# victorvg17/Towards-Interpretable-Reinforcement-Learning-Using-Attention-Augmented-Agents-Replication

Hardware: AMD Instinct MI355X
Metric: learner frames/sec (fwd+bwd, T=20 unroll) at 1/2/4/8 MI355X + % roofline (higher is better)
Workload: dtype fp32; 1 GPU; C2 (BASELINE.json configs[1]): B=32 per GPU x T=20 unroll, 84x84, 4 heads, fp32; global_batch=32, seq_len=20, frame=84x84, heads=4, parallelism=dp1

## Files before the change

### include/aaa.h

```cpp
#ifndef AAA_H
#define AAA_H

#include <stddef.h>
#include <hip/hip_runtime_api.h>

#ifdef __cplusplus
extern "C" {
#endif

#define AAA_ABI_VERSION 11

enum aaa_status {
  AAA_OK = 0,
  AAA_E_ARG = -1,
  AAA_E_ALIGN = -2,
  AAA_E_LAUNCH = -3,
  AAA_E_DEVICE = -4,
  AAA_E_STRANDED = -5
};

enum aaa_dtype {
  AAA_F32 = 0,
  AAA_BF16 = 1
};
// ... 171 lines not shown
  const void* packed;
  const float* basis;
  const void* frames;
  const float* prev_reward;
  const float* prev_action;
  float* h;
  float* c;
  float* logits;
  float* values;
  float* attn;
  void* workspace;
  unsigned long long seed;
  unsigned long long* counter;
  int* actions;
  float* logp;
  float* dlogp_dlogits;
  float* gates;
  float* h_out;
  float* c_out;
} aaa_actor_io;
size_t aaa_actor_workspace_bytes(const aaa_cfg* cfg);
int aaa_actor_step(const aaa_cfg* cfg, const aaa_actor_io* io, hipStream_t stream);

typedef struct aaa_actor_core_io {
  float* core_h;
  float* core_c;
  float* core_h_out;
  float* core_c_out;
  float* query;
} aaa_actor_core_io;
size_t aaa_actor_core_workspace_bytes(const aaa_cfg* cfg);
int aaa_actor_step_core(const aaa_cfg* cfg, const aaa_actor_io* io, const aaa_actor_core_io* core,
                        hipStream_t stream);


typedef struct aaa_conv_desc {
  int N, Hin, Win, Cin, Hout, Wout, Cout, KH, KW, stride, pad, dtype;
} aaa_conv_desc;

int aaa_conv2d_nhwc(const aaa_conv_desc* d, const float* x, const float* w, const float* bias,
                    float* y, hipStream_t stream);
int aaa_conv2d_nhwc_dgrad(const aaa_conv_desc* d, const float* dy, const float* w, float* dx,
                          hipStream_t stream);
int aaa_conv2d_nhwc_wgrad(const aaa_conv_desc* d, const float* x, const float* dy, float* dw,
                          hipStream_t stream);

int aaa_linear(int M, int N, int K, const float* x, const float* w, const float* bias, float* y,
               hipStream_t stream);


typedef struct aaa_cell_desc {
  int B, h, w, dtype;
} aaa_cell_desc;
size_t aaa_convlstm_packed_bytes(const aaa_cell_desc* d);
size_t aaa_convlstm_workspace_bytes(const aaa_cell_desc* d);
int aaa_convlstm_pack(const aaa_cell_desc* d, const float* cell_params, void* packed, hipStream_t stream);
int aaa_convlstm_cell_fwd(const aaa_cell_desc* d, const void* packed, const float* x, const float* h0,
                          const float* c0, float* h1, float* c1, void* workspace, hipStream_t stream);
int aaa_convlstm_cell_bwd(const aaa_cell_desc* d, const void* packed, const float* dh1, const float* dc1, float* dx,
                          float* dh0, float* dc0, float* cell_grads, void* workspace, hipStream_t stream);

typedef struct aaa_cnn_desc {
  int N, H, W, dtype;
} aaa_cnn_desc;
size_t aaa_vision_cnn_packed_bytes(const aaa_cnn_desc* d);
size_t aaa_vision_cnn_workspace_bytes(const aaa_cnn_desc* d);
int aaa_vision_cnn_pack(const aaa_cnn_desc* d, const float* cnn_params, void* packed, hipStream_t stream);
int aaa_vision_cnn_fwd(const aaa_cnn_desc* d, const float* cnn_params, const void* packed, const float* frames,
                       float* y1, float* y2, void* workspace, hipStream_t stream);
int aaa_vision_cnn_bwd(const aaa_cnn_desc* d, const void* packed, const float* dy2, float* dy1, float* cnn_grads,
                       void* workspace, hipStream_t stream);

typedef struct aaa_enc_desc {
  int N, H, W, dtype, flags, out_ld;
} aaa_enc_desc;
size_t aaa_vision_enc_workspace_bytes(const aaa_enc_desc* d);
int aaa_vision_enc_fwd(const aaa_enc_desc* d, const float* cnn_params, const void* packed, const void* frames,
                       void* xp, void* y1, void* out, hipStream_t stream);
int aaa_vision_enc_bwd(const aaa_enc_desc* d, const void* packed, const void* frames, const void* dy2,
                       const void* y1, void* xp, void* dy1, float* cnn_grads, int* fused, void* workspace,
                       hipStream_t stream);
int aaa_vision_enc_f32_fwd(const aaa_enc_desc* d, const float* cnn_params, const void* packed, const void* frames,
                           float* xp, float* y1, float* out, hipStream_t stream);

int aaa_attn_fwd(int F, int h, int w, int nq, const float* O, const float* S, const float* Q, int q_stride,
                 const float* prev_reward, const float* prev_action, float* attn, float* answer, hipStream_t stream);
int aaa_attn_bwd(int F, int h, int w, int nq, const float* O, const float* S, const float* Q, int q_stride,
                 const float* attn, const float* danswer, float* dO, float* dQ, hipStream_t stream);
int aaa_attn_fwd_bf16(int F, int h, int w, int nq, const void* O, int o_ld, const float* S, const float* Q,
                      int q_stride, float* sq_scratch, const float* prev_reward, const float* prev_action,
                      float* attn, float* answer, hipStream_t stream);
int aaa_attn_bwd_bf16(int F, int h, int w, int nq, const void* O, int o_ld, const float* S, const float* Q,
                      int q_stride, const float* attn, const float* danswer, int da_ld, int add_q,
                      int dO_quad_major, float* dO, float* dQ, hipStream_t stream);

int aaa_fastdiv_check(unsigned d, unsigned lo, unsigned hi, unsigned long long* mismatches);
int aaa_divisor_log(int enable, unsigned* out, int cap);

#ifdef __cplusplus
}
#endif
#endif
```

### towards-interpretable-reinforcement-learning-using-attention-augmented-agents-replication_amd/_native.py

```python
from __future__ import annotations

import ctypes
import os
import threading

_HERE = os.path.dirname(os.path.abspath(__file__))
LIB_PATH = os.environ.get("AAA_LIB") or os.path.join(_HERE, "libaaa.so")

F32, BF16 = 0, 1
ABI_VERSION = 11
E_STRANDED = -5
BWD_HEAD, BWD_CORE, BWD_VISION, BWD_ALL = 1, 2, 4, 7
FWD_VISION, FWD_CORE, FWD_TAIL, FWD_ALL = 1, 2, 4, 7

EXPORTS = (
    "aaa_abi_version", "aaa_last_error", "aaa_grid", "aaa_param_layout", "aaa_packed_bytes",
    "aaa_workspace_bytes", "aaa_pack_weights", "aaa_forward", "aaa_backward", "aaa_conv2d_nhwc",
    "aaa_conv2d_nhwc_dgrad", "aaa_conv2d_nhwc_wgrad", "aaa_linear", "aaa_timing_enable", "aaa_timing_read", "aaa_timing_stats",
    "aaa_adam_step", "aaa_reinforce", "aaa_sample_actions", "aaa_fastdiv_check", "aaa_divisor_log",
    "aaa_convlstm_packed_bytes", "aaa_convlstm_workspace_bytes", "aaa_convlstm_pack", "aaa_convlstm_cell_fwd",
    "aaa_convlstm_cell_bwd", "aaa_vision_cnn_packed_bytes", "aaa_vision_cnn_workspace_bytes", "aaa_vision_cnn_pack",
    "aaa_vision_cnn_fwd", "aaa_vision_cnn_bwd", "aaa_attn_fwd", "aaa_attn_bwd", "aaa_attn_fwd_bf16", "aaa_attn_bwd_bf16",
    "aaa_actor_workspace_bytes", "aaa_actor_step", "aaa_pair_status", "aaa_pair_flag", "aaa_pair_flag_at",
    "aaa_adam_step_guarded", "aaa_adam_step_counted", "aaa_workspace_region",
    "aaa_core_elem_bytes", "aaa_forward_phases", "aaa_core_export", "aaa_core_import",
    "aaa_actor_core_workspace_bytes", "aaa_actor_step_core",
    "aaa_vision_enc_workspace_bytes", "aaa_vision_enc_fwd", "aaa_vision_enc_bwd",
    "aaa_vtrace",
    "aaa_forward_resets", "aaa_backward_resets",
    "aaa_vision_enc_f32_fwd",
    "aaa_grad_norm_scratch_bytes", "aaa_grad_norm", "aaa_grad_scale", "aaa_adam_step_clipped",
)
TIMER_FWD_STEP, TIMER_BPTT_STEP, TIMER_CORE_WGRAD, TIMER_ATTN_FWD, TIMER_ATTN_BWD = 0, 1, 2, 3, 4
TIMER_PACK, TIMER_VISION_FWD, TIMER_TAIL_FWD, TIMER_TAIL_BWD, TIMER_CORE_DX, TIMER_VISION_BWD, TIMER_MISC = range(5, 12)
TIMER_N = 12


class Cfg(ctypes.Structure):
    _fields_ = [("B", ctypes.c_int), ("T", ctypes.c_int), ("H", ctypes.c_int), ("W", ctypes.c_int),
                ("nq", ctypes.c_int), ("A", ctypes.c_int), ("dtype", ctypes.c_int), ("flags", ctypes.c_int)]


IO_FIELDS = ("params", "packed", "basis", "frames", "prev_reward", "prev_action", "h0", "c0",
             "logits", "values", "attn", "hT", "cT", "dlogits", "dvalues", "dhT", "dcT",
             "grads", "dh0", "dc0", "workspace",
             "core_h0", "core_c0", "core_hT", "core_cT", "dcore_hT", "dcore_cT", "dcore_h0", "dcore_c0")
FLAG_STATEFUL_CORE = 1
FLAG_FRAMES_U8 = 2
FLAG_DEFER_STRANDED = 4
WS_ANSWER_HIDDEN, WS_QUERY_HIDDEN0, WS_QUERY_HIDDEN1 = 0, 1, 2
WS_CORE_XH, WS_CORE_DO, WS_CORE_DX = 3, 4, 5


class TimerStats(ctypes.Structure):
    _fields_ = [("total_ms", ctypes.c_double), ("launches", ctypes.c_long), ("work", ctypes.c_double),
                ("variant", ctypes.c_char * 192)]


class IO(ctypes.Structure):
    _fields_ = [(n, ctypes.c_void_p) for n in IO_FIELDS]


ACTOR_IO_FIELDS = ("params", "packed", "basis", "frames", "prev_reward", "prev_action", "h", "c",
                   "logits", "values", "attn", "workspace")


class ActorIO(ctypes.Structure):
    _fields_ = [(n, ctypes.c_void_p) for n in ACTOR_IO_FIELDS] + [
        ("seed", ctypes.c_ulonglong), ("counter", ctypes.c_void_p), ("actions", ctypes.c_void_p),
        ("logp", ctypes.c_void_p), ("dlogp_dlogits", ctypes.c_void_p), ("gates", ctypes.c_void_p),
        ("h_out", ctypes.c_void_p), ("c_out", ctypes.c_void_p)]


class ActorCoreIO(ctypes.Structure):
    _fields_ = [(n, ctypes.c_void_p) for n in ("core_h", "core_c", "core_h_out", "core_c_out", "query")]


class VtraceDesc(ctypes.Structure):
    _fields_ = [(n, ctypes.c_int) for n in ("T", "B", "A", "value_col")] + [
        (n, ctypes.c_double) for n in ("gamma", "lam", "rho_bar", "c_bar", "pg_rho_bar", "baseline_cost",
                                       "entropy_cost", "scale")]


VTRACE_IO_FIELDS = ("logits", "values", "actions", "rewards", "behaviour_logp", "done", "bootstrap",
                    "dlogits", "dvalues", "vs", "pg_adv", "loss")


class VtraceIO(ctypes.Structure):
    _fields_ = [(n, ctypes.c_void_p) for n in VTRACE_IO_FIELDS]


class AdamHP(ctypes.Structure):
    _fields_ = [("lr", ctypes.c_double), ("beta1", ctypes.c_double), ("beta2", ctypes.c_double),
                ("eps", ctypes.c_double), ("weight_decay", ctypes.c_double), ("amsgrad", ctypes.c_int),
                ("maximize", ctypes.c_int)]


class CellDesc(ctypes.Structure):
    _fields_ = [(n, ctypes.c_int) for n in ("B", "h", "w", "dtype")]


class CnnDesc(ctypes.Structure):
    _fields_ = [(n, ctypes.c_int) for n in ("N", "H", "W", "dtype")]


class EncDesc(ctypes.Structure):
    _fields_ = [(n, ctypes.c_int) for n in ("N", "H", "W", "dtype", "flags", "out_ld")]


class ConvDesc(ctypes.Structure):
    _fields_ = [(n, ctypes.c_int) for n in
                ("N", "Hin", "Win", "Cin", "Hout", "Wout", "Cout", "KH", "KW", "stride", "pad", "dtype")]


_lib = None
_lock = threading.Lock()


def ablation_build() -> bool:
    return hasattr(load(), "aaa_ablation_build")


def load(path: str = LIB_PATH):
    global _lib
    with _lock:
        if _lib is not None:
            return _lib
        if not os.path.isfile(path):
            raise RuntimeError(f"aaa: native library {path} is missing; build it with "
                               f"`make -C {os.path.join(_HERE, 'csrc')}` -- there is no CPU fallback")
        lib = ctypes.CDLL(path)
        P, I, S = ctypes.c_void_p, ctypes.c_int, ctypes.c_size_t
        CP = ctypes.POINTER(Cfg)
        sig = {
            "aaa_abi_version": (I, []),
            "aaa_last_error": (ctypes.c_char_p, []),
            "aaa_grid": (I, [I, I, ctypes.POINTER(I), ctypes.POINTER(I)]),
            "aaa_param_layout": (I, [CP, ctypes.POINTER(S), ctypes.POINTER(S), ctypes.POINTER(S)]),
            "aaa_packed_bytes": (S, [CP]),
            "aaa_workspace_bytes": (S, [CP]),
            "aaa_pack_weights": (I, [CP, P, P, P]),
            "aaa_forward": (I, [CP, ctypes.POINTER(IO), P]),
            "aaa_backward": (I, [CP, ctypes.POINTER(IO), I, P]),
            "aaa_forward_phases": (I, [CP, ctypes.POINTER(IO), I, P]),
            "aaa_forward_resets": (I, [CP, ctypes.POINTER(IO), I, P, P]),
            "aaa_backward_resets": (I, [CP, ctypes.POINTER(IO), I, P, P]),
            "aaa_core_export": (I, [CP, P, I, I, P, P, P, P]),
            "aaa_core_import": (I, [CP, P, I, I, P, P, P, P]),
            "aaa_conv2d_nhwc": (I, [ctypes.POINTER(ConvDesc), P, P, P, P, P]),
            "aaa_conv2d_nhwc_dgrad": (I, [ctypes.POINTER(ConvDesc), P, P, P, P]),
            "aaa_conv2d_nhwc_wgrad": (I, [ctypes.POINTER(ConvDesc), P, P, P, P]),
            "aaa_linear": (I, [I, I, I, P, P, P, P, P]),
            "aaa_timing_enable": (I, [I]),
            "aaa_timing_read": (I, [I, ctypes.POINTER(ctypes.c_double), ctypes.POINTER(ctypes.c_long)]),
            "aaa_timing_stats": (I, [I, ctypes.POINTER(TimerStats)]),
            "aaa_adam_step": (I, [ctypes.POINTER(AdamHP), ctypes.c_long, I, P, P, P, P, P, P, P]),
            "aaa_adam_step_guarded": (I, [ctypes.POINTER(AdamHP), ctypes.c_long, P, I, P, P, P, P, P, P, P]),
            "aaa_pair_flag": (I, [P, P]),
            "aaa_pair_flag_at": (I, [P, P, P]),
            "aaa_adam_step_counted": (I, [ctypes.POINTER(AdamHP), P, P, I, P, P, P, P, P, P, P]),
            "aaa_grad_norm_scratch_bytes": (S, [I, P]),
            "aaa_grad_norm": (I, [ctypes.c_double, I, P, P, P, P, P]),
            "aaa_grad_scale": (I, [P, I, P, P, P]),
            "aaa_adam_step_clipped": (I, [ctypes.POINTER(AdamHP), P, P, P, I, P, P, P, P, P, P, P]),
            "aaa_core_elem_bytes": (I, [ctypes.POINTER(Cfg), ctypes.POINTER(I), ctypes.POINTER(I)]),
            "aaa_workspace_region": (I, [ctypes.POINTER(Cfg), I, ctypes.POINTER(ctypes.c_size_t),
                                         ctypes.POINTER(ctypes.c_size_t)]),
            "aaa_reinforce": (I, [I, I, I, P, P, P, ctypes.c_double, P, P, P, P]),
            "aaa_vtrace": (I, [ctypes.POINTER(VtraceDesc), ctypes.POINTER(VtraceIO), P]),
            "aaa_sample_actions": (I, [I, I, P, ctypes.c_ulonglong, P, P, P, P, P]),
            "aaa_convlstm_packed_bytes": (S, [ctypes.POINTER(CellDesc)]),
            "aaa_convlstm_workspace_bytes": (S, [ctypes.POINTER(CellDesc)]),
            "aaa_convlstm_pack": (I, [ctypes.POINTER(CellDesc), P, P, P]),
            "aaa_convlstm_cell_fwd": (I, [ctypes.POINTER(CellDesc), P, P, P, P, P, P, P, P]),
            "aaa_convlstm_cell_bwd": (I, [ctypes.POINTER(CellDesc), P, P, P, P, P, P, P, P, P]),
            "aaa_vision_cnn_packed_bytes": (S, [ctypes.POINTER(CnnDesc)]),
            "aaa_vision_cnn_workspace_bytes": (S, [ctypes.POINTER(CnnDesc)]),
            "aaa_vision_cnn_pack": (I, [ctypes.POINTER(CnnDesc), P, P, P]),
            "aaa_vision_cnn_fwd": (I, [ctypes.POINTER(CnnDesc), P, P, P, P, P, P, P]),
            "aaa_vision_cnn_bwd": (I, [ctypes.POINTER(CnnDesc), P, P, P, P, P, P]),
            "aaa_vision_enc_workspace_bytes": (S, [ctypes.POINTER(EncDesc)]),
            "aaa_vision_enc_fwd": (I, [ctypes.POINTER(EncDesc), P, P, P, P, P, P, P]),
            "aaa_vision_enc_bwd": (I, [ctypes.POINTER(EncDesc), P, P, P, P, P, P, P, ctypes.POINTER(I), P, P]),
            "aaa_vision_enc_f32_fwd": (I, [ctypes.POINTER(EncDesc), P, P, P, P, P, P, P]),
            "aaa_attn_fwd": (I, [I, I, I, I, P, P, P, I, P, P, P, P, P]),
            "aaa_attn_bwd": (I, [I, I, I, I, P, P, P, I, P, P, P, P, P]),
            "aaa_attn_fwd_bf16": (I, [I, I, I, I, P, I, P, P, I, P, P, P, P, P, P]),
            "aaa_attn_bwd_bf16": (I, [I, I, I, I, P, I, P, P, I, P, P, I, I, I, P, P, P]),
            "aaa_fastdiv_check": (I, [ctypes.c_uint, ctypes.c_uint, ctypes.c_uint, ctypes.POINTER(ctypes.c_ulonglong)]),
            "aaa_divisor_log": (I, [I, ctypes.POINTER(ctypes.c_uint), I]),
            "aaa_actor_workspace_bytes": (S, [CP]),
            "aaa_actor_step": (I, [CP, ctypes.POINTER(ActorIO), P]),
            "aaa_actor_core_workspace_bytes": (S, [CP]),
            "aaa_actor_step_core": (I, [CP, ctypes.POINTER(ActorIO), ctypes.POINTER(ActorCoreIO), P]),
            "aaa_pair_status": (I, [P, I]),
        }
        ab_override = "AAA_LIB" in os.environ
        missing = [name for name in sig if not hasattr(lib, name)]
        if missing and not ab_override:
            raise RuntimeError(f"aaa: {path} does not export {missing}; it is older than these bindings -- "
                               f"rebuild it (make -C {os.path.join(_HERE, 'csrc')})")
        for name, (res, args) in sig.items():
            if name in missing:
                continue
            fn = getattr(lib, name)
            fn.restype, fn.argtypes = res, args
        abi = lib.aaa_abi_version()
        if abi != ABI_VERSION and not ab_override:
            raise RuntimeError(f"aaa: {path} has ABI version {abi}, these bindings expect {ABI_VERSION}; "
                               f"rebuild it (make -C {os.path.join(_HERE, 'csrc')})")
        _lib = lib
        return lib


def check(rc: int, what: str = "") -> None:
    if rc != 0:
        msg = load().aaa_last_error().decode(errors="replace")
        raise RuntimeError(f"aaa{(' ' + what) if what else ''}: {msg} (status {rc})")


def ptr(t) -> int | None:
    if t is None:
        return None
    return t.data_ptr()


def stream_ptr(device=None) -> int:
    import torch
    return torch.cuda.current_stream(device).cuda_stream


def grid(H: int, W: int):
    h, w = ctypes.c_int(), ctypes.c_int()
    check(load().aaa_grid(H, W, ctypes.byref(h), ctypes.byref(w)), "grid")
    return h.value, w.value


def param_layout(cfg: Cfg):
    total = ctypes.c_size_t()
    offs = (ctypes.c_size_t * 34)()
    sizes = (ctypes.c_size_t * 34)()
    check(load().aaa_param_layout(ctypes.byref(cfg), ctypes.byref(total), offs, sizes), "param_layout")
    return total.value, list(offs), list(sizes)


def fastdiv_check(d: int, lo: int = 0, hi: int = 1 << 31) -> int:
    bad = ctypes.c_ulonglong()
    check(load().aaa_fastdiv_check(d, lo, hi, ctypes.byref(bad)), "fastdiv_check")
    return bad.value


def divisor_log(enable: int = -1):
    n = load().aaa_divisor_log(-1, None, 0)
    buf = (ctypes.c_uint * max(n, 1))()
    n = load().aaa_divisor_log(enable, buf, n)
    return sorted(set(buf[:n]))


def timing_enable(on: bool = True) -> None:
    check(load().aaa_timing_enable(1 if on else 0), "timing_enable")


def timing_read(kind: int):
    ms, n = ctypes.c_double(), ctypes.c_long()
    check(load().aaa_timing_read(kind, ctypes.byref(ms), ctypes.byref(n)), "timing_read")
    return ms.value, n.value

# ... 85 lines not shown
```

### towards-interpretable-reinforcement-learning-using-attention-augmented-agents-replication_amd/csrc/misc.h

```cpp
#pragma once
#include "common.h"
#include "epilogues.h"

namespace aaa {

struct LstmPtrs {
  const float* wx[4];
  const float* bx[4];
  const float* wh[4];
};
struct LstmGrads {
  float* wx[4];
  float* bx[4];
  float* wh[4];
};
struct F32Pack {
  const float *a0w, *wih, *bih, *bhh, *pw, *vw, *pb, *vb;
  float *W1p, *Wihp, *blc, *Whd, *bhd;
  int ans_in, ans_ld, A, ldy;
  const float* whh = nullptr;
  float* Wihhp = nullptr;
};
struct F32Unpack {
  const float *gW1p, *gWihp, *gblc, *gWhd, *gbhd;
  float *a0w, *wih, *bih, *bhh, *pw, *vw, *pb, *vb;
  int ans_in, ans_ld, A;
  const float* gWihhp = nullptr;
  float* whh = nullptr;
};

template <typename T>
struct PackAll {
  const float *c1w, *c2w;
  T *Wp1, *Wp2, *WdT2;
  LstmPtrs lstm;
  T *WpX, *WpH, *WdT, *WpXH;
  float* bl;
  F32Pack f32;
  __bf16 *W1s = nullptr, *W2s = nullptr;
};
template <typename T> hipError_t pack_all(const PackAll<T>& a, hipStream_t st);
hipError_t pack_vis_split(const float* c1w, const float* c2w, __bf16* W1s, __bf16* W2s, hipStream_t st);

hipError_t query_pack(const float* b0, const float* W2, const float* b2, const float* W4, const float* b4, int nq,
                      float* q1, float* q2, float* Q, hipStream_t st);
hipError_t query_sq(const float* S, const float* Q, int P, int nq, float* SQ, hipStream_t st);
struct OSrc {
  const void* p;
  int bf16, ld;
  OSrc frame(size_t f, int P) const {
    return {(const char*)p + f * P * ld * (bf16 ? 2 : 4), bf16, ld};
  }
};
inline OSrc o_f32(const float* Hs) { return {Hs, 0, 128}; }
inline OSrc o_bf16(const __bf16* h, int ld) { return {h, 1, ld}; }
hipError_t attn_fwd(OSrc O, const float* S, const float* Q, const float* SQ, const float* pr,
                    const float* pa, int F, int P, int nq, float* Am, float* ans, int ans_ld, hipStream_t st,
                    int qs = 0);
hipError_t attn_bwd(OSrc O, const float* S, const float* Q, const float* Am, const float* dAns,
                    int da_ld, int F, int P, int nq, float* dO, float* dQp, hipStream_t st, int qs = 0,
                    int addq = 0, int cqm = 0);
hipError_t cqm_convert(const float* src, float* dst, int nf, int P, int to_cqm, hipStream_t st);
hipError_t query_bwd(const float* dQs, const float* gb1, const float* W1, int ans_in, int nq, const float* W2,
                     const float* W4, const float* q1, const float* q2, float* gW4, float* gb4, float* gW2,
                     float* gb2, float* gb0, hipStream_t st);
struct ColSumSeg {
  const float* X;
  int ld, N;
  float* out;
};
struct ColSums {
  ColSumSeg s[6];
  int n = 0;
  int cb[7];
  void add(const float* X, int ld, int N, float* out) { s[n++] = ColSumSeg{X, ld, N, out}; }
};
hipError_t colsum_multi(ColSums c, int M, hipStream_t st);
template <typename TI> hipError_t colsum(const TI* X, int ld, int M, int N, float* out, hipStream_t st);
template <typename TZ, typename GT>
hipError_t gate_bwd_last(int M, int bj, const float* dO, const float* dhT, const GT* gates, const float* cprev,
                         const float* ccur, float* dC, TZ* dz, float* part, hipStream_t st, int nsl = 1,
                         size_t sls = 0);
hipError_t concat_dy(int F, int A, int ldy, const float* dl, const float* dv, float* dY, hipStream_t st);
struct ZeroRanges {
  float* p[4];
  long n[4];
  int cnt;
  void add(float* q, long m) {
    if (q && m > 0) { p[cnt] = q; n[cnt] = m; ++cnt; }
  }
};
template <typename T>
hipError_t prologue(const ZeroRanges& z, int M, const float* h0, T* xh, int F, int A, int ldy, const float* dl,
                    const float* dv, float* dY, hipStream_t st);
template <typename T> hipError_t state_to_xh(int M, const float* h0, T* xh, hipStream_t st);
template <typename T> hipError_t xh_to_state(int M, const T* xh, float* h, hipStream_t st);
template <typename T> hipError_t cell_xh(int M, const float* x, const float* h, T* xh, hipStream_t st);
template <typename TI, typename TO> hipError_t cast(long n, const TI* src, TO* dst, hipStream_t st);
template <typename T> hipError_t pack_conv(const float* w, int Cout, int Cin, int K, T* dst, hipStream_t st);
template <typename T>
hipError_t pack_lstm_all(const LstmPtrs& L, T* WpX, T* WpH, T* WdT, float* bl, T* WpXH, hipStream_t st);
template <typename T>
hipError_t gate_fwd_zx(int M, const float* cprev, float* gates, float* cnext, float* hout, T* xhnext, hipStream_t st,
                       const float* zs = nullptr, int nsl = 0, size_t sls = 0, const float* bias = nullptr);
struct ResetZero { float* p; int ld, w, es; };
struct ResetZeros {
  ResetZero r[4];
  int n = 0;
  ResetZeros& add(float* p, int ld, int w, int es = 1) {
    if (p) r[n++] = ResetZero{p, ld, w, es};
    return *this;
  }
};
hipError_t reset_rows(const float* rs, int B, int rpb, const ResetZeros& z, const float* src, float* dst, int cw,
                      hipStream_t st);
hipError_t reset_gate_bwd(const float* rs_in, const float* rs_c, int M, int P, const float* dO, const float* gates,
                          const float* cprev, const float* ccur, float* dC, float* dz, hipStream_t st);
hipError_t pack_f32(const F32Pack& p, hipStream_t st);
hipError_t reorder_cmaj(const float* src, int rows, int Cin, int taps, int BK, float* dst, hipStream_t st);
hipError_t split_planes(const float* src, long n, __bf16* dst, hipStream_t st);
template <typename T, typename TI> hipError_t frames_rgbx(int F, int H, int W, const TI* x, T* y, hipStream_t st);
template <typename T> hipError_t pack_conv2_classes(const float* w2, T* dst, hipStream_t st);
template <typename T> hipError_t pack_conv1_rgbx(const float* w, T* dst, hipStream_t st);
hipError_t unpack_conv1_rgbx(const float* g, float* dst, hipStream_t st);
hipError_t unpack_conv(const float* g, int Cout, int Cin, int K, float* dst, hipStream_t st);
// ... 7 lines not shown
```

### towards-interpretable-reinforcement-learning-using-attention-augmented-agents-replication_amd/csrc/misc.hip

```cpp
#include <cstdlib>
#include <type_traits>

#include "misc.h"

namespace aaa {

__device__ __forceinline__ float wave_sum(float v) {
#pragma unroll
  for (int o = 32; o > 0; o >>= 1) v += __shfl_xor(v, o, 64);
  return v;
}
__device__ __forceinline__ void lds_barrier() { asm volatile("s_waitcnt lgkmcnt(0)\n\ts_barrier" ::: "memory"); }
__device__ __forceinline__ float wave_max(float v) {
#pragma unroll
  for (int o = 32; o > 0; o >>= 1) v = fmaxf(v, __shfl_xor(v, o, 64));
  return v;
}

__global__ void k_gemv_cols_atomic(const float* __restrict__ W, int ldw, const float* __restrict__ x, int N, int K,
                                   int rows_per, float* y) {
  const int o0 = blockIdx.x * rows_per, o1 = min(N, o0 + rows_per);
  for (int k = threadIdx.x; k < K; k += blockDim.x) {
    float s = 0.f;
#pragma unroll 8
// ... 793 lines not shown
        }
    } else {
      z = *reinterpret_cast<const f32x4*>(gates + (size_t)m * 512 + 4 * ch);
    }
    float gi, gf, gc, go, c, h;
    GateFwd::run(z[0], z[1], z[2], z[3], cprev[idx], gi, gf, gc, go, c, h);
    cnext[idx] = c;
    if (hout) hout[idx] = h;
    xhnext[(size_t)m * 192 + 64 + ch] = (T)h;
    *reinterpret_cast<f32x4*>(gates + (size_t)m * 512 + 4 * ch) = f32x4{gi, gf, gc, go};
  }
}

__host__ __device__ inline int pack_f32_n(const F32Pack& p) {
  return 512 * p.ans_ld + 1024 * 256 + 1024 + p.ldy * 256 + p.ldy + (p.Wihhp ? 1024 * 512 : 0);
}
__device__ __forceinline__ void pack_f32_el(int idx, const F32Pack& p) {
  const int n1 = 512 * p.ans_ld, n2 = 1024 * 256, n3 = 1024, n4 = p.ldy * 256, n5 = p.ldy;
  int i = idx;
  if (i >= n1 + n2 + n3 + n4 + n5) {
    i -= n1 + n2 + n3 + n4 + n5;
    const int row = i >> 9, k = i & 511, u = row >> 2, g = row & 3;
    p.Wihhp[i] = k < 256 ? p.wih[(size_t)(g * 256 + u) * 256 + k] : p.whh[(size_t)(g * 256 + u) * 256 + k - 256];
    return;
  }
  if (i < n1) {
    const int o = i / p.ans_ld, k = i - o * p.ans_ld;
    p.W1p[i] = k < p.ans_in ? p.a0w[(size_t)o * p.ans_in + k] : 0.f;
    return;
  }
  i -= n1;
  if (i < n2) {
    const int row = i >> 8, k = i & 255, u = row >> 2, g = row & 3;
    p.Wihp[i] = p.wih[(size_t)(g * 256 + u) * 256 + k];
    return;
  }
  i -= n2;
  if (i < n3) {
    const int u = i >> 2, g = i & 3;
    p.blc[i] = p.bih[g * 256 + u] + p.bhh[g * 256 + u];
    return;
  }
  i -= n3;
  if (i < n4) {
    const int o = i >> 8, k = i & 255;
    float v = 0.f;
    if (o < p.A) v = p.pw[o * 256 + k];
    else if (o < 2 * p.A) v = p.vw[(o - p.A) * 256 + k];
    p.Whd[i] = v;
    return;
  }
  i -= n4;
  float v = 0.f;
  if (i < p.A) v = p.pb[i];
  else if (i < 2 * p.A) v = p.vb[i - p.A];
  p.bhd[i] = v;
}
__global__ void k_pack_f32(F32Pack p) {
  const int tot = pack_f32_n(p);
  for (int idx = blockIdx.x * blockDim.x + threadIdx.x; idx < tot; idx += gridDim.x * blockDim.x) pack_f32_el(idx, p);
}

__device__ __forceinline__ void vis_split_el(float v, int row, int k, int nks, __bf16* dst) {
  const __bf16 hi = (__bf16)v;
  const float r = v - (float)hi;
  const __bf16 mid = (__bf16)r;
  const __bf16 lo = (__bf16)(r - (float)mid);
  const size_t o = ((size_t)(((row >> 5) * nks + (k >> 4)) * 3) * 64 + ((k >> 3) & 1) * 32 + (row & 31)) * 8 + (k & 7);
  dst[o] = hi;
  dst[o + 512] = mid;
  dst[o + 1024] = lo;
}
__global__ void k_pack_vis_split(const float* __restrict__ c1w, const float* __restrict__ c2w, __bf16* W1s, __bf16* W2s) {
  const int n1 = 32 * 256, tot = n1 + 64 * 512;
  for (int idx = blockIdx.x * blockDim.x + threadIdx.x; idx < tot; idx += gridDim.x * blockDim.x) {
    if (idx < n1) {
      vis_split_el(pack_conv1_rgbx_val(idx, c1w), idx >> 8, idx & 255, 16, W1s);
    } else {
      const int i = idx - n1;
      vis_split_el(pack_conv_val(i, c2w, 32, 4), i >> 9, i & 511, 32, W2s);
    }
  }
}

template <typename T>
__global__ void k_pack_all(PackAll<T> a) {
  const int n1 = 32 * 256, n2 = n1 + 64 * 512, n3 = n2 + 4 * 32 * 256, n4 = n3 + kPackLstmN;
  const int tot = n4 + pack_f32_n(a.f32);
  for (int idx = blockIdx.x * blockDim.x + threadIdx.x; idx < tot; idx += gridDim.x * blockDim.x) {
    if (idx < n1) {
      pack_conv1_rgbx_el(idx, a.c1w, a.Wp1);
      if constexpr (std::is_same<T, float>::value)
        if (a.W1s) vis_split_el(a.Wp1[idx], idx >> 8, idx & 255, 16, a.W1s);
    } else if (idx < n2) {
      pack_conv_el(idx - n1, a.c2w, 32, 4, a.Wp2);
      if constexpr (std::is_same<T, float>::value)
        if (a.W2s) vis_split_el(a.Wp2[idx - n1], (idx - n1) >> 9, (idx - n1) & 511, 32, a.W2s);
    }
    else if (idx < n3) pack_conv2_classes_el(idx - n2, a.c2w, a.WdT2);
    else if (idx < n4) pack_lstm_el(idx - n3, a.lstm, a.WpX, a.WpH, a.bl, a.WdT, a.WpXH);
    else pack_f32_el(idx - n4, a.f32);
  }
}


__device__ __forceinline__ void unpack_conv_el(int idx, const float* __restrict__ g, int Cin, int K, float* dst) {
  int r = idx;
  const int ky = r % K; r /= K;
  const int kx = r % K; r /= K;
  const int ci = r % Cin, o = r / Cin;
  dst[idx] = g[(size_t)o * K * K * Cin + (ky * K + kx) * Cin + ci];
}
__global__ void k_unpack_conv(const float* __restrict__ g, int Cout, int Cin, int K, float* dst) {
  const int n = Cout * Cin * K * K;
  for (int idx = blockIdx.x * blockDim.x + threadIdx.x; idx < n; idx += gridDim.x * blockDim.x)
    unpack_conv_el(idx, g, Cin, K, dst);
}

constexpr int kUnpackLstmN = 4 * (128 * 64 * 9 + 128 * 128 * 9 + 128);
__device__ __forceinline__ void unpack_lstm_el(int idx, const float* __restrict__ gW, const float* __restrict__ gb,
                                               const LstmGrads& L) {
  const int nx = 128 * 64 * 9, nh = 128 * 128 * 9;
  {
    const int per = nx + nh + 128;
    const int g = idx / per;
    int i = idx - g * per;
    if (i < nx) {
      int r = i;
      const int ky = r % 3; r /= 3;
      const int kx = r % 3; r /= 3;
      const int ci = r % 64, ch = r / 64;
      L.wx[g][i] = gW[(size_t)(4 * ch + g) * 1728 + (ky * 3 + kx) * 192 + ci];
    } else if ((i -= nx) < nh) {
      int r = i;
      const int ky = r % 3; r /= 3;
      const int kx = r % 3; r /= 3;
      const int ci = r % 128, ch = r / 128;
      L.wh[g][i] = gW[(size_t)(4 * ch + g) * 1728 + (ky * 3 + kx) * 192 + 64 + ci];
    } else {
      i -= nh;
      L.bx[g][i] = gb[4 * i + g];
    }
  }
}
__global__ void k_unpack_lstm(const float* __restrict__ gW, const float* __restrict__ gb, LstmGrads L) {
  for (int idx = blockIdx.x * blockDim.x + threadIdx.x; idx < kUnpackLstmN; idx += gridDim.x * blockDim.x)
    unpack_lstm_el(idx, gW, gb, L);
}
__global__ void k_unpack_cv(const float* __restrict__ gW, const float* __restrict__ gb, LstmGrads L,
                            const float* __restrict__ g2, float* d2, const float* __restrict__ g1, float* d1) {
  const int n0 = gW ? kUnpackLstmN : 0, n1 = n0 + 64 * 32 * 16, n2 = n1 + 32 * 3 * 64;
  for (int idx = blockIdx.x * blockDim.x + threadIdx.x; idx < n2; idx += gridDim.x * blockDim.x) {
    if (idx < n0) unpack_lstm_el(idx, gW, gb, L);
    else if (idx < n1) unpack_conv_el(idx - n0, g2, 32, 4, d2);
    else unpack_conv1_rgbx_el(idx - n1, g1, d1);
  }
}

__global__ void k_unpack_f32(F32Unpack p) {
  const int n1 = 512 * p.ans_in, n2 = 1024 * 256, n3 = 1024, n4 = 2 * p.A * 256, n5 = 2 * p.A;
  const int tot = n1 + n2 + n3 + n4 + n5;
  for (int idx = blockIdx.x * blockDim.x + threadIdx.x; idx < tot; idx += gridDim.x * blockDim.x) {
    int i = idx;
    if (i < n1) {
      const int o = i / p.ans_in, k = i - o * p.ans_in;
      p.a0w[i] = p.gW1p[(size_t)o * p.ans_ld + k];
      continue;
    }
    i -= n1;
    if (i < n2) {
      const int row = i >> 8, k = i & 255, g = row >> 8, u = row & 255;
      if (p.gWihhp) {
        p.wih[i] = p.gWihhp[(size_t)(4 * u + g) * 512 + k];
        p.whh[i] = p.gWihhp[(size_t)(4 * u + g) * 512 + 256 + k];
      } else {
        p.wih[i] = p.gWihp[(size_t)(4 * u + g) * 256 + k];
      }
      continue;
    }
    i -= n2;
    if (i < n3) {
      const int g = i >> 8, u = i & 255;
// ... 287 lines not shown
}

hipError_t unpack_conv(const float* g, int Cout, int Cin, int K, float* dst, hipStream_t st) {
  hipLaunchKernelGGL(k_unpack_conv, dim3(nblk((long)Cout * Cin * K * K)), dim3(256), 0, st, g, Cout, Cin, K, dst);
  return hipGetLastError();
}

hipError_t unpack_lstm(const float* gW, const float* gb, const LstmGrads& L, hipStream_t st) {
  hipLaunchKernelGGL(k_unpack_lstm, dim3(nblk(4L * (128 * 64 * 9 + 128 * 128 * 9 + 128))), dim3(256), 0, st, gW,
                     gb, L);
  return hipGetLastError();
}

hipError_t unpack_f32(const F32Unpack& p, hipStream_t st) {
  long n = 512L * p.ans_in + 1024L * 256 + 1024 + 2L * p.A * 256 + 2 * p.A;
  hipLaunchKernelGGL(k_unpack_f32, dim3(nblk(n)), dim3(256), 0, st, p);
  return hipGetLastError();
}

template <typename T, typename TI>
hipError_t frames_rgbx(int F, int H, int W, const TI* x, T* y, hipStream_t st) {
  hipLaunchKernelGGL((k_frames_rgbx<T, TI>), dim3(nblk((long)F * (H + 2) * (W + 2))), dim3(256), 0, st, F, H, W, x, y);
  return hipGetLastError();
}
template <typename T>
hipError_t pack_conv2_classes(const float* w2, T* dst, hipStream_t st) {
  hipLaunchKernelGGL(k_pack_conv2_classes<T>, dim3(nblk(4 * 32 * 256)), dim3(256), 0, st, w2, dst);
  return hipGetLastError();
}
template <typename T>
hipError_t pack_conv1_rgbx(const float* w, T* dst, hipStream_t st) {
  hipLaunchKernelGGL(k_pack_conv1_rgbx<T>, dim3(nblk(32 * 256)), dim3(256), 0, st, w, dst);
  return hipGetLastError();
}
hipError_t unpack_conv1_rgbx(const float* g, float* dst, hipStream_t st) {
  hipLaunchKernelGGL(k_unpack_conv1_rgbx, dim3(nblk(32 * 3 * 64)), dim3(256), 0, st, g, dst);
  return hipGetLastError();
}
template hipError_t colsum<float>(const float*, int, int, int, float*, hipStream_t);
template hipError_t colsum<__bf16>(const __bf16*, int, int, int, float*, hipStream_t);
template hipError_t gate_bwd_last<float, float>(int, int, const float*, const float*, const float*, const float*,
                                                const float*, float*, float*, float*, hipStream_t, int, size_t);
template hipError_t gate_bwd_last<__bf16, float>(int, int, const float*, const float*, const float*, const float*,
                                                 const float*, float*, __bf16*, float*, hipStream_t, int, size_t);
template hipError_t gate_bwd_last<float, _Float16>(int, int, const float*, const float*, const _Float16*,
                                                   const float*, const float*, float*, float*, float*, hipStream_t, int, size_t);
template hipError_t gate_bwd_last<__bf16, _Float16>(int, int, const float*, const float*, const _Float16*,
                                                    const float*, const float*, float*, __bf16*, float*, hipStream_t, int, size_t);
template hipError_t frames_rgbx<float, float>(int, int, int, const float*, float*, hipStream_t);
template hipError_t frames_rgbx<__bf16, float>(int, int, int, const float*, __bf16*, hipStream_t);
template hipError_t frames_rgbx<float, uint8_t>(int, int, int, const uint8_t*, float*, hipStream_t);
template hipError_t frames_rgbx<__bf16, uint8_t>(int, int, int, const uint8_t*, __bf16*, hipStream_t);
template hipError_t pack_conv2_classes<float>(const float*, float*, hipStream_t);
template hipError_t pack_conv2_classes<__bf16>(const float*, __bf16*, hipStream_t);
template hipError_t pack_conv1_rgbx<float>(const float*, float*, hipStream_t);
template hipError_t pack_conv1_rgbx<__bf16>(const float*, __bf16*, hipStream_t);
template hipError_t cell_xh<float>(int, const float*, const float*, float*, hipStream_t);
template hipError_t cell_xh<__bf16>(int, const float*, const float*, __bf16*, hipStream_t);
template hipError_t cast<float, __bf16>(long, const float*, __bf16*, hipStream_t);
template hipError_t cast<__bf16, float>(long, const __bf16*, float*, hipStream_t);
template hipError_t cast<float, float>(long, const float*, float*, hipStream_t);
template hipError_t state_to_xh<float>(int, const float*, float*, hipStream_t);
template hipError_t state_to_xh<__bf16>(int, const float*, __bf16*, hipStream_t);
template hipError_t prologue<float>(const ZeroRanges&, int, const float*, float*, int, int, int, const float*,
                                    const float*, float*, hipStream_t);
template hipError_t prologue<__bf16>(const ZeroRanges&, int, const float*, __bf16*, int, int, int, const float*,
                                     const float*, float*, hipStream_t);
template hipError_t xh_to_state<__bf16>(int, const __bf16*, float*, hipStream_t);
template hipError_t pack_conv<float>(const float*, int, int, int, float*, hipStream_t);
template hipError_t pack_conv<__bf16>(const float*, int, int, int, __bf16*, hipStream_t);
template hipError_t pack_lstm_all<float>(const LstmPtrs&, float*, float*, float*, float*, float*, hipStream_t);
template hipError_t pack_lstm_all<__bf16>(const LstmPtrs&, __bf16*, __bf16*, __bf16*, float*, __bf16*, hipStream_t);
template hipError_t gate_fwd_zx<float>(int, const float*, float*, float*, float*, float*, hipStream_t, const float*, int, size_t,
                                         const float*);
template hipError_t gate_fwd_zx<__bf16>(int, const float*, float*, float*, float*, __bf16*, hipStream_t, const float*, int, size_t,
                                         const float*);

template <typename T>
hipError_t pack_all(const PackAll<T>& a, hipStream_t st) {
  const long n = 32L * 256 + 64 * 512 + 4 * 32 * 256 + kPackLstmN + pack_f32_n(a.f32);
  hipLaunchKernelGGL(k_pack_all<T>, dim3(nblk(n)), dim3(256), 0, st, a);
  return hipGetLastError();
}
hipError_t pack_vis_split(const float* c1w, const float* c2w, __bf16* W1s, __bf16* W2s, hipStream_t st) {
  hipLaunchKernelGGL(k_pack_vis_split, dim3(nblk(32L * 256 + 64 * 512)), dim3(256), 0, st, c1w, c2w, W1s, W2s);
  return hipGetLastError();
}
template hipError_t pack_all<float>(const PackAll<float>&, hipStream_t);
template hipError_t pack_all<__bf16>(const PackAll<__bf16>&, hipStream_t);

hipError_t unpack_cv(const float* gW, const float* gb, const LstmGrads& L, const float* g2, float* d2, const float* g1,
                     float* d1, hipStream_t st) {
  const long n = (gW ? kUnpackLstmN : 0) + 64L * 32 * 16 + 32 * 3 * 64;
  hipLaunchKernelGGL(k_unpack_cv, dim3(nblk(n)), dim3(256), 0, st, gW, gb, L, g2, d2, g1, d1);
  return hipGetLastError();
}

__global__ void k_colsum_multi(ColSums c, int M, int rows_per) {
  __shared__ float red[256];
  int k = 0;
  while (k + 1 < c.n && (int)blockIdx.x >= c.cb[k + 1]) ++k;
  const ColSumSeg s = c.s[k];
  const int col = ((int)blockIdx.x - c.cb[k]) * 64 + (threadIdx.x & 63);
  const int r0 = blockIdx.y * rows_per, r1 = min(M, r0 + rows_per);
  float acc = 0.f;
  if (col < s.N) {
#pragma unroll 8
    for (int r = r0 + (threadIdx.x >> 6); r < r1; r += 4) acc += s.X[(size_t)r * s.ld + col];
  }
  red[threadIdx.x] = acc;
  __syncthreads();
  if (threadIdx.x < 64 && col < s.N)
    atomicAdd(s.out + col, red[threadIdx.x] + red[threadIdx.x + 64] + red[threadIdx.x + 128] + red[threadIdx.x + 192]);
}

hipError_t colsum_multi(ColSums c, int M, hipStream_t st) {
  if (M <= 0 || c.n <= 0) return hipSuccess;
  c.cb[0] = 0;
  for (int k = 0; k < c.n; ++k) c.cb[k + 1] = c.cb[k] + (c.s[k].N + 63) / 64;
  const int cols = c.cb[c.n];
  int split = (1024 + cols - 1) / cols;
  int rows_per = (M + split - 1) / split;
  if (rows_per < 64) rows_per = 64;
  split = (M + rows_per - 1) / rows_per;
  hipLaunchKernelGGL(k_colsum_multi, dim3(cols, split), dim3(256), 0, st, c, M, rows_per);
  return hipGetLastError();
}

}
```

### towards-interpretable-reinforcement-learning-using-attention-augmented-agents-replication_amd/csrc/rt.h

```cpp
#pragma once
#include <algorithm>
#include <cstdarg>
#include <cstdio>
#include <cstring>
#include <cstdlib>
#include <memory>
#include <mutex>
#include <string>
#include <thread>
#include <type_traits>
#include <utility>
#include <vector>

#include "aaa.h"
#include "epilogues.h"
#include "gemm.h"
#include "loaders_b.h"
#include "glds.h"
#include "gemm_deep.h"
#include "halo.h"
#include "recur.h"
#include "recur_bwd.h"
#include "recur_f32.h"
#include "recur_bwd_f32.h"
#include "vision.h"
#include "vision_f32.h"
#include "vision_bwd.h"
#include "misc.h"
#include "optim.h"
#include "actor.h"
#include "step_tiles.h"


namespace aaa {

extern thread_local std::string g_err;

int fail(int code, const char* fmt, ...);

#define HIPCHK(expr)                                                                      \
  do {                                                                                    \
    hipError_t e_ = (expr);                                                               \
    if (e_ != hipSuccess)                                                                 \
      return fail(AAA_E_LAUNCH, "%s failed: %s (%s:%d)", #expr, hipGetErrorString(e_),   \
                  __FILE__, __LINE__);                                                    \
  } while (0)

inline size_t al256(size_t x) { return (x + 255) & ~size_t(255); }
inline int cdiv(int a, int b) { return (a + b - 1) / b; }
inline int conv_out(int n, int k, int s, int p) {
  const int d = n + 2 * p - k;
  return d < 0 ? 0 : d / s + 1;
}

enum PIdx {
  C0W = 0, C0B, C1W, C1B,
  XI_W, XI_B, HI_W, XF_W, XF_B, HF_W, XC_W, XC_B, HC_W, XO_W, XO_B, HO_W,
  Q0W, Q0B, Q2W, Q2B, Q4W, Q4B, A0W, A0B, A2W, A2B, WIH, WHH, BIH, BHH, PW, PB, VW, VB, NPARAM
};

struct Layout {
  int B, T, F, H, W, H1, W1, P1, h, w, P, nq, A, dt, esz;
  int sc;
  int fu8;
  int fchunk;
  int xpc;
  int qd, da, ans_in, ans_ld, ldy;
  size_t poff[NPARAM], psz[NPARAM], ptotal;
  size_t k_Wp1, k_Wp2, k_WdT2, k_W1s, k_W2s, k_WpX, k_WpH, k_WpXH, k_Wfr, k_Wbf, k_Wf32, k_Wb32, k_Wf6, k_Wf6p, k_Wb6, k_Wx6, k_Wb6p, k_Wx6p, k_WdTl, k_WdTc, k_WdT6, k_bl, k_Wihhp, k_q1, k_q2, k_Q, k_W1p, k_Wihp, k_blc, k_Whd, k_bhd, packed;
  size_t Xp, Y1, XH, Hs, Cst, Gt, SQ, Am, ans, hid1, AO, LG, LC, LH;
  size_t dY, dLG, dAO, dH1, dAns, dO, dQp, dQs, dC, dZ, dZp, dY2, dY1, dxb, rflags, xpart, dhs, dZ6;
  size_t gWp1, gWp2, gWpl, gbl, gW1p, gWihp, gblc, gWhd, gbhd, ws;
  size_t CH, CC, AOX, Qf, q1s, q2s, dAOX, dQf, dq2s, dq1s, dhc, dcc, gWihhp;
};

inline double vision_fwd_flop(const Layout& L) { return 2.0 * L.P1 * 32 * 192 + 2.0 * L.P * 64 * 512; }
inline double tail_fwd_flop(const Layout& L) {
  return 2.0 * ((double)L.ans_in * 512 + 512.0 * 256 + 256.0 * 1024);
}
inline double vision_bwd_flop(const Layout& L) { return 2.0 * (2.0 * L.P * 64 * 512) + 2.0 * L.P1 * 32 * 192; }

int build_layout(const aaa_cfg* c, Layout& L, int min_frames = 0);
int check_device();

inline bool aligned16(const void* p) { return ((uintptr_t)p & 15) == 0; }

int pair_budget(int T);
int* pair_report(int dev);
int* pair_flag_base(int dev);
int pair_take();
int pair_peek();
int pair_check();
inline int report_word(const char* what, int** rep) {
  int dev = 0;
  HIPCHK(hipGetDevice(&dev));
  if (!(*rep = pair_report(dev))) return fail(AAA_E_LAUNCH, "cannot map the %s report word", what);
  return AAA_OK;
}

hipStream_t aux_stream();
hipStream_t side_stream();
hipError_t record_event(hipStream_t s, hipEvent_t* out);
hipError_t stream_order(hipStream_t from, hipStream_t to);

struct Timers {
  std::mutex mu;
  bool on = false;
  std::vector<std::pair<hipEvent_t, hipEvent_t>> pending[AAA_TIMER_N];
  double work[AAA_TIMER_N] = {};
  std::string variant[AAA_TIMER_N];
  std::vector<hipEvent_t> pool;
  hipEvent_t get() {
    if (!pool.empty()) { hipEvent_t e = pool.back(); pool.pop_back(); return e; }
    hipEvent_t e = nullptr;
    if (hipEventCreate(&e) != hipSuccess) return nullptr;
    return e;
  }
};
extern Timers g_timers;

struct TimerScope {
  int kind;
  hipStream_t st;
  hipEvent_t a = nullptr, b = nullptr;
  double work;
  std::string variant;
  TimerScope(int k, hipStream_t s, double w, std::string v) : kind(k), st(s), work(w), variant(std::move(v)) {
    std::lock_guard<std::mutex> lk(g_timers.mu);
    if (!g_timers.on) return;
    a = g_timers.get();
    b = g_timers.get();
    if (a && b) (void)hipEventRecord(a, st);
  }
  ~TimerScope() {
    if (!a || !b) return;
    (void)hipEventRecord(b, st);
    std::lock_guard<std::mutex> lk(g_timers.mu);
    g_timers.pending[kind].emplace_back(a, b);
    g_timers.work[kind] += work;
    g_timers.variant[kind] = variant;
  }
};

std::string strf(const char* fmt, ...);

inline double attn_fwd_bytes(int P, int nq, int ans_ld, int oesz = 4) {
  return oesz * 128.0 * P + 4.0 * (nq * P + ans_ld);
}
inline double attn_bwd_bytes(int P, int nq, int oesz = 4) {
  return oesz * 128.0 * P + 4.0 * (128.0 * P + nq * P + 184.0 * nq + 72.0 * nq);
}

// ... 211 lines not shown

static bool pipe_batched() { return env_int("AAA_PIPE_BATCHED", 1) != 0; }

static int wgrad_splits(int tiles, int K, int BK) {
  int s = std::max(1, 1024 / std::max(tiles, 1));
  int maxs = std::max(1, K / (8 * BK));
  return std::min(s, maxs);
}

static int fused_splitk() { return std::max(2, std::min(4, env_int("AAA_FUSED_SPLITK", 3))); }
static int splitk_nbuf() { return std::max(2, std::min(4, ab_int("AAA_SPLITK_NBUF", 2))); }
template <class CK, class EP, typename T>
static hipError_t step_gemm_splitk(const T* W, int ldw, int wrows, const T* src, const ConvGeo& g, int M,
                                   uint32_t src_bytes, const EP& ep, int Mi, int K, hipStream_t st, int nsplit,
                                   bool ilv = false) {
  switch (splitk_nbuf() * 2 + (ilv ? 1 : 0)) {
    case 4: return step_gemm<CK, true, T, T, EP, 2, false>(W, ldw, wrows, src, g, M, src_bytes, ep, Mi, K, st, nsplit);
    case 5: return step_gemm<CK, true, T, T, EP, 2, true>(W, ldw, wrows, src, g, M, src_bytes, ep, Mi, K, st, nsplit);
    case 6: return step_gemm<CK, true, T, T, EP, 3, false>(W, ldw, wrows, src, g, M, src_bytes, ep, Mi, K, st, nsplit);
    case 7: return step_gemm<CK, true, T, T, EP, 3, true>(W, ldw, wrows, src, g, M, src_bytes, ep, Mi, K, st, nsplit);
    case 8: return step_gemm<CK, true, T, T, EP, 4, false>(W, ldw, wrows, src, g, M, src_bytes, ep, Mi, K, st, nsplit);
    default: return step_gemm<CK, true, T, T, EP, 4, true>(W, ldw, wrows, src, g, M, src_bytes, ep, Mi, K, st, nsplit);
  }
}
template <typename T, typename GT>
static int fused_step(const T* WpXH, const T* xht, int h, int w, int M, const EpiConvLstmFwd<T, GT>& ep,
                      hipStream_t st, float* zpart = nullptr, bool resets = false) {
  using EF = EpiConvLstmFwd<T, GT>;
  const ConvGeo g = ConvGeo{192, 192, 0, h, w, h, w, 3, 1, 1, 0}.prep();
  const uint32_t xh_bytes = (uint32_t)((size_t)M * 192 * sizeof(T));
  constexpr bool f32 = std::is_same<T, float>::value;
  const int want = env_int("AAA_FUSED_TILE", f32 ? (f32_split6() ? (zpart ? 18 : 13) : 4) : 9);
  const int ftile = tile_dt(FusedTiles{}, want) ? want : 4;
  if (ftile != want && !tile_known(want)) return tile_unknown("AAA_FUSED_TILE");
  return for_tile<FusedTiles>(ftile, (int)AAA_E_ARG, [&](auto tile) -> int {
    using Tl = decltype(tile);
    using CK = typename Tl::template Cfg<T>;
    constexpr bool slices = Tl::split == SplitK::Slices;
    TimerScope tim(AAA_TIMER_FWD_STEP, st, 2.0 * M * 512 * 1728,
                   strf("%s fused [x|h] step, K=1728, AAA_FUSED_TILE %d%s [kernel: EpiConvLstmFwd]%s", f32 ? "fp32" : "bf16",
                        ftile, f32 && Tl::split_product && !slices ? " (bf16x6 split products)" : "",
                        resets ? ", resets" : ""));
    if constexpr (!Tl::template serves<T, GT>()) {
      return fail(AAA_E_ARG, "AAA_FUSED_TILE %d: fp32 split-product tiles only", ftile);
    } else if constexpr (slices) {
      if (!zpart || !ep.bias) return fail(AAA_E_ARG, "AAA_FUSED_TILE %d: split-K needs B*P < 8192 (got %d)", ftile, M);
      const int ns = splitk_slices(1728, CK::BK, fused_splitk());
      const EpiSliceT es{zpart, 512, 512, M, (size_t)M * 512};
      HIPCHK((step_gemm_splitk<CK>(WpXH, 1728, 512, xht, g, M, xh_bytes, es, 512, 1728, st, ns, Tl::ILV)));
      HIPCHK(gate_fwd_zx<typename CK::type>(M, ep.cprev, ep.gates, ep.cnext, ep.hout, ep.xhnext, st, zpart, ns,
                                            (size_t)M * 512, ep.bias));
    } else {
      HIPCHK((step_gemm<CK, Tl::stage != Stage::Reg, T, T, EF, Tl::NBUF, Tl::ILV>(WpXH, 1728, 512, xht, g, M, xh_bytes, ep, 512,
                                                                                  1728, st)));
    }
    return AAA_OK;
  });
}

int device_cus();
int frames_g(const Layout& L, const char* env);
int frames_band(const Layout& L);
int f32_frames(const Layout& L);
int frames_bwd(const Layout& L, bool g16);
int cqm_layout(const Layout& L);
inline OSrc readout_h(const Layout& L, char* ws) {
  if (L.esz == 2) return o_bf16((const __bf16*)(ws + L.XH) + (size_t)L.B * L.P * 192 + 64, 192);
  return o_f32((const float*)(ws + L.Hs));
}
int rec_stagger(const char* env);
bool f32_split6();

template <typename T> int pack_impl(const Layout& L, const float* prm, char* pk, hipStream_t st);
template <typename T, typename OT>
int vision_fwd(const Layout& L, int F, const char* pk, const float* prm, const void* frames, T* Xp, T* Y1, OT* out,
               int out_ld, hipStream_t st, bool xp_full = true, std::string* ran = nullptr);
template <typename T>
int forward_impl(const Layout& L, const aaa_io* io, hipStream_t st, int phases, const float* reset = nullptr);
template <typename T>
int lstm_wgrad(const T* dz, const T* xh, int rows, int h, int w, float* gW, hipStream_t s, bool aux);
template <typename T>
int vision_bwd(const Layout& L, const char* pk, const T* dy2, const T* y1, T* xp, T* dy1, int F, float* gW2,
               float* gW1, float* gb1, hipStream_t s, const void* frames = nullptr);
const char* vision_bwd_variant(bool fused);
template <typename T>
int vision_bwd_alone(const Layout& L, const char* pk, const void* frames, const T* dy2, const T* y1, T* xp, T* dy1,
                     void* part, size_t part_bytes, int F, float* gW2, float* gW1, float* gb1, hipStream_t st,
                     const void* xp_frames, bool* fused);
template <typename T>
int backward_impl(const Layout& L, const aaa_io* io, int phases, hipStream_t st, const float* reset = nullptr);

}
```

### towards-interpretable-reinforcement-learning-using-attention-augmented-agents-replication_amd/csrc/rt_backward.hip

```cpp
#include "rt.h"

namespace aaa {


template <typename T>
static int conv2_dgrad(const Layout& L, const char* pk, const T* dy2, T* dy1, int frames, float* gbias,
                       hipStream_t s) {
  {
    constexpr int CKd = std::is_same<T, float>::value ? 32 : 64;
    const int Ha = (L.H1 + 1) / 2, Wa = (L.W1 + 1) / 2;
    auto halo4 = [&](auto cfg, auto nbuf) -> int {
      using HC = decltype(cfg);
      EpiStoreParity4<T> ep(dy1, frames * Ha * Wa, Ha, Wa, L.H1, L.W1, gbias);
      const HaloParams hp{pk + L.k_WdT2, 256, 128, dy2, 64, 0, 64, (uint32_t)((size_t)frames * L.P * 64 * L.esz),
                          L.h, L.w, frames, 0, Ha, Wa};
      HIPCHK((launch_halo<HC, EpiStoreParity4<T>, 2, decltype(nbuf)::value>(hp, ep, s)));
      return AAA_OK;
    };
    using NB3 = std::integral_constant<int, 3>;
    auto fits = [&](int fr, int bj, int hmax) {
      return fr * Ha * Wa <= bj && fr * (L.h + 2) * (L.w + 2) + 1 <= hmax && Ha <= L.h && Wa <= L.w;
    };
    const int fr = ab_int("AAA_DGRAD2_FR", std::is_same<T, float>::value ? 1 : 2);
    if (ab_int("AAA_DGRAD2_HALO", 1)) {
// ... 238 lines not shown
          rc = wgrad_lstm_pipe(GemmCfg<T, 256, 256, 32, 2, 4>{}, I3{}, I2{});
        break;
      case 8:
        if constexpr (std::is_same<T, float>::value)
          rc = wgrad_lstm_pipe(GemmCfg<T, 128, 128, WBK, 2, 2>{}, I3{}, I2{});
        else
          rc = wgrad_lstm_pipe(GemmCfg<T, 256, 256, 32, 2, 2>{}, std::integral_constant<int, 4>{}, I2{});
        break;
      case 9:
        if constexpr (std::is_same<T, float>::value)
          rc = wgrad_lstm_pipe(GemmCfg<T, 128, 128, WBK, 2, 2>{}, I3{}, I2{});
        else
          rc = wgrad_lstm_pipe(GemmCfg<T, 256, 256, 32, 2, 4>{}, std::integral_constant<int, 4>{},
                               std::integral_constant<int, kReadAhead>{});
        break;
      default: rc = wgrad_lstm_pipe(GemmCfg<T, 128, 128, WBK, 2, 2>{}, I2{}, I0{}); break;
    }
    if (rc) return rc;
  } else if (std::is_same<T, float>::value && f32_split6()) {
    auto s6 = [&](auto cfg) {
      using CS6 = std::conditional_t<std::is_same<T, float>::value, decltype(cfg), CfgWFor<T>>;
      return wgrad_lstm(CS6{});
    };
#ifdef AAA_ABLATION
    const int tile6 = ab_int("AAA_WGRAD_S6_TILE", 6);
    const int rc = tile6 == 1   ? s6(GemmCfgS6<128, 256, 32, 2, 2>{})
                   : tile6 == 2 ? s6(GemmCfgS6<256, 128, 32, 2, 2>{})
                   : tile6 == 3 ? s6(GemmCfgS6<256, 256, 32, 2, 4>{})
                   : tile6 == 4 ? s6(GemmCfgS6L<256, 256, 16, 2, 4>{})
                   : tile6 == 5 ? s6(GemmCfgS6L<256, 128, 16, 2, 2>{})
                   : tile6 == 6 ? s6(GemmCfgS6L<256, 256, 16, 2, 4, 2>{})
                   : tile6 == 7 ? s6(GemmCfgS6L<256, 192, 16, 4, 2, 2>{})
                                : s6(GemmCfgS6<128, 128, 32, 2, 2>{});
#else
    const int rc = s6(GemmCfgS6L<256, 256, 16, 2, 4, 2>{});
#endif
    if (rc) return rc;
  } else {
    const int wide = ab_int("AAA_AUX_WIDE", aux ? 0 : 1);
#ifdef AAA_ABLATION
    const int rc = !wide ? wgrad_lstm(CfgFor<T>{})
                   : ab_int("AAA_WGRAD_TILE", 0) == 1 ? wgrad_lstm(GemmCfg<T, 128, 192, 32, 2, 2>{})
                                                       : wgrad_lstm(CfgWFor<T>{});
#else
    const int rc = !wide ? wgrad_lstm(CfgFor<T>{}) : wgrad_lstm(CfgWFor<T>{});
#endif
    if (rc) return rc;
  }
  return AAA_OK;
}

template <typename T>
static int conv1_wgrad_frames(const Layout& L, const T* dy1, const void* frames, int n, T* xpbuf, float* gW,
                              hipStream_t s) {
  const size_t fb = (size_t)L.H * L.W * 3 * (L.fu8 ? 1 : 4);
  for (int s0 = 0; s0 < n; s0 += L.xpc) {
    const int m = std::min(L.xpc, n - s0);
    const char* fr = (const char*)frames + (size_t)s0 * fb;
    if (L.fu8) HIPCHK((frames_rgbx<T, uint8_t>(m, L.H, L.W, (const uint8_t*)fr, xpbuf, s)));
    else HIPCHK((frames_rgbx<T, float>(m, L.H, L.W, (const float*)fr, xpbuf, s)));
    const int rc = conv1_wgrad<T>(L, dy1 + (size_t)s0 * L.P1 * 32, xpbuf, m, gW, s);
    if (rc) return rc;
  }
  return AAA_OK;
}

template <typename T>
int vision_bwd(const Layout& L, const char* pk, const T* dy2, const T* y1, T* xp, T* dy1, int F,
                      float* gW2, float* gW1, float* gb1, hipStream_t s, const void* frames) {
  const size_t fb = (size_t)L.H * L.W * 3 * (L.fu8 ? 1 : 4);
  for (int f0 = 0; f0 < F; f0 += L.fchunk) {
    const int n = std::min(L.fchunk, F - f0);
    const T* d2 = dy2 + (size_t)f0 * L.P * 64;
    T* d1 = dy1 + (size_t)f0 * L.P1 * 32;
    int rc = conv2_wgrad<T>(L, d2, y1 + (size_t)f0 * L.P1 * 32, n, gW2, s);
    if (!rc) rc = conv2_dgrad<T>(L, pk, d2, d1, n, gb1, s);
    if (!rc && frames) rc = conv1_wgrad_frames<T>(L, d1, (const char*)frames + (size_t)f0 * fb, n, xp, gW1, s);
    else if (!rc) rc = conv1_wgrad<T>(L, d1, xp + (size_t)f0 * (L.H + 2) * (L.W + 2) * 4, n, gW1, s);
    if (rc) return rc;
  }
  return AAA_OK;
}

template <typename T>
static bool vbwd_on(const Layout& L, int F, size_t part_bytes = 0) {
  if constexpr (!std::is_same<T, __bf16>::value) {
    (void)L; (void)F; (void)part_bytes;
    return false;
  } else {
    if (!part_bytes) part_bytes = (size_t)F * L.P1 * 32 * L.esz;
    return L.fu8 && vbwd_fits(L.H, L.W, L.H1, L.W1, L.h, L.w) && env_int("AAA_VIS_FRAMES", 1) &&
           env_int("AAA_VIS_BWD_FRAMES", 1) && F >= env_int("AAA_VBWD_MINF", 0) * device_cus() &&
           (size_t)vbwd_groups(F, device_cus()) * kVbPart * 4 <= part_bytes;
  }
}
template <typename T>
static int vbwd_run(const Layout& L, const char* pk, const void* frames, int f0, int F, const T* dy2, const T* y1,
                    T* dy1, float* gW2, float* gW1, float* gb1, hipStream_t s) {
  if constexpr (!std::is_same<T, __bf16>::value) {
    return fail(AAA_E_ARG, "the frame-resident vision backward is bf16 only");
  } else {
    VisBwdParams vp{(const char*)frames + (size_t)f0 * L.H * L.W * 3 * (L.fu8 ? 1 : 4), dy2, y1,
                    (const __bf16*)(pk + L.k_WdT2), (float*)dy1, F, L.H, L.W, L.H1, L.W1, L.h, L.w};
    HIPCHK(vision_bwd_frames(vp, device_cus(), gW2, gW1, gb1, s));
    return AAA_OK;
  }
}

const char* vision_bwd_variant(bool fused) {
  return fused ? "frame-resident conv2 wgrad + dgrad + conv1 wgrad [kernel: k_vision_bwd_frames], grad unpack"
               : "conv2 wgrad + dgrad, conv1 wgrad, grad unpack";
}
template <typename T>
int vision_bwd_alone(const Layout& L, const char* pk, const void* frames, const T* dy2, const T* y1, T* xp, T* dy1,
                     void* part, size_t part_bytes, int F, float* gW2, float* gW1, float* gb1, hipStream_t st,
                     const void* xp_frames, bool* fused) {
  const bool on = vbwd_on<T>(L, F, part_bytes);
  if (fused) *fused = on;
  if (on) return vbwd_run<T>(L, pk, frames, 0, F, dy2, y1, part ? (T*)part : dy1, gW2, gW1, gb1, st);
  const int rc = vision_bwd<T>(L, pk, dy2, y1, xp, dy1, F, gW2, gW1, gb1, st, xp_frames);
  if (rc) return rc;
  if (std::is_same<T, float>::value && !ab_int("AAA_CONV2_DGRAD_RING", 1))
    HIPCHK(colsum(dy1, 32, F * L.P1, 32, gb1, st));
  return AAA_OK;
}

struct BwdCtx {
  const Layout& L;
  const aaa_io* io;
  char* ws;
  const char* pk;
  const float* prm;
  float* grads;
  hipStream_t st;
  const float* reset;
  float* Wf(size_t off) const { return (float*)(ws + off); }
  template <typename T> T* Wt(size_t off) const { return (T*)(ws + off); }
};

template <class EP>
static hipError_t tail_dgrad(const Rows& Wt, const Rows& dY, const EP& ep, int Mi, int Nj, int K, hipStream_t st) {
  return head_gemm<LdRowsT, LdRows>(Wt, dY, ep, Mi, Nj, K, 1, st);
}
static hipError_t tail_wgrad(const Rows& dA, const Rows& X, float* out, int ldo, int F, hipStream_t st) {
  const int Mi = dA.nrows, Nj = X.nrows;
  return head_gemm<LdRowsT, LdRowsT>(dA, X, EpiStore<true>{out, ldo, Mi, Nj}, Mi, Nj, F,
                                     wgrad_splits(cdiv(Mi, 64) * cdiv(Nj, 64), F, CF::BK), st);
}
static hipError_t tail_unpack(const Layout& L, char* ws, float* grads, bool stateful, hipStream_t st) {
  auto Wf = [&](size_t off) { return (float*)(ws + off); };
  F32Unpack up;
  up.gW1p = Wf(L.gW1p); up.gWihp = Wf(L.gWihp); up.gblc = Wf(L.gblc); up.gWhd = Wf(L.gWhd); up.gbhd = Wf(L.gbhd);
  up.a0w = grads + L.poff[A0W]; up.wih = grads + L.poff[WIH]; up.bih = grads + L.poff[BIH];
  up.bhh = grads + L.poff[BHH]; up.pw = grads + L.poff[PW]; up.vw = grads + L.poff[VW];
  up.pb = grads + L.poff[PB]; up.vb = grads + L.poff[VB];
  up.ans_in = L.ans_in; up.ans_ld = L.ans_ld; up.A = L.A;
  if (stateful) {
    up.gWihhp = Wf(L.gWihhp);
    up.whh = grads + L.poff[WHH];
  }
  return unpack_f32(up, st);
}

static int head_backward_stateful(const BwdCtx& c) {
  const Layout& L = c.L;
  const aaa_io* io = c.io;
  const hipStream_t st = c.st;
  const float *prm = c.prm, *reset = c.reset;
  float* grads = c.grads;
  const int F = L.F, P = L.P, B = L.B, qd = L.qd, da = L.da;
  float *CH = c.Wf(L.CH), *CC = c.Wf(L.CC), *AOX = c.Wf(L.AOX), *dAOX = c.Wf(L.dAOX), *dhc = c.Wf(L.dhc),
        *dcc = c.Wf(L.dcc);
  const size_t sB = (size_t)B * 256 * 4;
  if (io->dcore_hT) HIPCHK(hipMemcpyAsync(dhc, io->dcore_hT, sB, hipMemcpyDeviceToDevice, st));
  else HIPCHK(hipMemsetAsync(dhc, 0, sB, st));
  if (io->dcore_cT) HIPCHK(hipMemcpyAsync(dcc, io->dcore_cT, sB, hipMemcpyDeviceToDevice, st));
  else HIPCHK(hipMemsetAsync(dcc, 0, sB, st));
  for (int t = L.T - 1; t >= 0; --t) {
    const size_t f0 = (size_t)t * B;
    float *dLG = c.Wf(L.dLG) + f0 * 1024, *dH1 = c.Wf(L.dH1) + f0 * 512, *dAns = c.Wf(L.dAns) + f0 * da;
    float *dQf = c.Wf(L.dQf) + f0 * qd, *dq2 = c.Wf(L.dq2s) + f0 * qd, *dq1 = c.Wf(L.dq1s) + f0 * 128;
    HIPCHK(tail_dgrad({(const float*)(c.pk + L.k_Whd), 256, 256}, {c.Wf(L.dY) + f0 * L.ldy, L.ldy, B},
                      EpiLstmCellBwdS{c.Wf(L.LG) + f0 * 1024, CC + f0 * 256, CC + (f0 + B) * 256, dhc, dcc, dLG, B}, 256,
                      B, L.ldy, st));
    if (reset)
      HIPCHK(reset_rows(reset + f0, B, 1, ResetZeros{}.add(dLG + 1, 1024, 256, 4).add(dcc, 256, 256), nullptr, nullptr,
                        0, st));
    HIPCHK(tail_dgrad({(const float*)(c.pk + L.k_Wihhp), 512, 512}, {dLG, 1024, B},
                      EpiStoreT<float>{dAOX + f0 * 512, 512, 512, B, nullptr, 0}, 512, B, 1024, st));
    HIPCHK(tail_dgrad({prm + L.poff[A2W], 512, 512}, {dAOX + f0 * 512, 512, B},
                      EpiReluBwdT{dH1, c.Wf(L.hid1) + f0 * 512, 512, 512, 512, B}, 512, B, 256, st));
    HIPCHK(tail_dgrad({(const float*)(c.pk + L.k_W1p), L.ans_ld, da}, {dH1, 512, B},
                      EpiStoreT<float>{dAns, da, da, B, nullptr, 0}, da, B, 512, st));
    {
      TimerScope tim(AAA_TIMER_ATTN_BWD, st, (double)B * attn_bwd_bytes(P, L.nq, L.esz), "k_attn_bwd, per-frame query (stateful core)");
      HIPCHK(attn_bwd(readout_h(L, c.ws).frame(f0, P), io->basis, c.Wf(L.Qf) + f0 * qd, c.Wf(L.Am) + f0 * P * L.nq, dAns,
                      da, B, P, L.nq, c.Wf(L.dO) + f0 * P * 128, dQf, st, qd, 1, (cqm_layout(L) & kCqmDO) != 0));
    }
    HIPCHK(tail_dgrad({prm + L.poff[Q4W], qd, qd}, {dQf, qd, B},
                      EpiReluBwdT{dq2, c.Wf(L.q2s) + f0 * qd, qd, qd, qd, B}, qd, B, qd, st));
    HIPCHK(tail_dgrad({prm + L.poff[Q2W], 128, 128}, {dq2, qd, B},
                      EpiReluBwdT{dq1, c.Wf(L.q1s) + f0 * 128, 128, 128, 128, B}, 128, B, qd, st));
// ... 13 lines not shown
  HIPCHK(tail_wgrad({c.Wf(L.dH1), 512, 512}, {c.Wf(L.ans), L.ans_ld, L.ans_ld}, c.Wf(L.gW1p), L.ans_ld, F, st));
  HIPCHK(colsum(c.Wf(L.dH1), 512, F, 512, grads + L.poff[A0B], st));
  HIPCHK(tail_wgrad({c.Wf(L.dQf), qd, qd}, {c.Wf(L.q2s), qd, qd}, grads + L.poff[Q4W], qd, F, st));
  HIPCHK(colsum(c.Wf(L.dQf), qd, F, qd, grads + L.poff[Q4B], st));
  HIPCHK(tail_wgrad({c.Wf(L.dq2s), qd, qd}, {c.Wf(L.q1s), 128, 128}, grads + L.poff[Q2W], 128, F, st));
  HIPCHK(colsum(c.Wf(L.dq2s), qd, F, qd, grads + L.poff[Q2B], st));
  HIPCHK(tail_wgrad({c.Wf(L.dq1s), 128, 128}, reset ? Rows{AOX + 256, 512, 256} : Rows{CH, 256, 256},
                    grads + L.poff[Q0W], 256, F, st));
  HIPCHK(colsum(c.Wf(L.dq1s), 128, F, 128, grads + L.poff[Q0B], st));
  HIPCHK(tail_unpack(L, c.ws, grads, true, st));
  return AAA_OK;
}

static int head_backward_zero_state(const BwdCtx& c) {
  const Layout& L = c.L;
  const hipStream_t st = c.st;
  const float* prm = c.prm;
  float* grads = c.grads;
  const int F = L.F, P = L.P;
  std::unique_ptr<TimerScope> tail(new TimerScope(AAA_TIMER_TAIL_BWD, st, 2.0 * F * (tail_fwd_flop(L) + 2.0 * 256 * L.ldy),
                                                  "heads + LSTMCell + answer MLP backward (fp32 GEMMs)"));
  hipStream_t ss = F >= 2048 ? side_stream() : nullptr;
  hipStream_t ws_ = ss ? ss : st;
  if (ss) HIPCHK(stream_order(st, ss));
  HIPCHK(tail_wgrad({c.Wf(L.dY), L.ldy, L.ldy}, {c.Wf(L.LH), 256, 256}, c.Wf(L.gWhd), 256, F, ws_));
  HIPCHK(tail_dgrad({(const float*)(c.pk + L.k_Whd), 256, 256}, {c.Wf(L.dY), L.ldy, F},
                    EpiLstmCellBwd{c.Wf(L.LG), c.Wf(L.LC), c.Wf(L.dLG), F}, 256, F, L.ldy, st));
  if (ss) HIPCHK(stream_order(st, ss));
  HIPCHK(tail_wgrad({c.Wf(L.dLG), 1024, 1024}, {c.Wf(L.AO), 256, 256}, c.Wf(L.gWihp), 256, F, ws_));
  HIPCHK(tail_dgrad({(const float*)(c.pk + L.k_Wihp), 256, 256}, {c.Wf(L.dLG), 1024, F},
                    EpiStoreT<float>{c.Wf(L.dAO), 256, 256, F, nullptr, 0}, 256, F, 1024, st));
  if (ss) HIPCHK(stream_order(st, ss));
  HIPCHK(tail_wgrad({c.Wf(L.dAO), 256, 256}, {c.Wf(L.hid1), 512, 512}, grads + L.poff[A2W], 512, F, ws_));
  HIPCHK(tail_dgrad({prm + L.poff[A2W], 512, 512}, {c.Wf(L.dAO), 256, F},
                    EpiReluBwdT{c.Wf(L.dH1), c.Wf(L.hid1), 512, 512, 512, F}, 512, F, 256, st));
  if (ss) HIPCHK(stream_order(st, ss));
  HIPCHK(tail_wgrad({c.Wf(L.dH1), 512, 512}, {c.Wf(L.ans), L.ans_ld, L.ans_ld}, c.Wf(L.gW1p), L.ans_ld, F, ws_));
  HIPCHK(tail_dgrad({(const float*)(c.pk + L.k_W1p), L.ans_ld, L.da}, {c.Wf(L.dH1), 512, F},
                    EpiStoreT<float>{c.Wf(L.dAns), L.da, L.da, F, nullptr, 0}, L.da, F, 512, st));
  tail.reset();
  {
    TimerScope tim(AAA_TIMER_ATTN_BWD, st, (double)F * attn_bwd_bytes(P, L.nq, L.esz), "k_attn_bwd, 1 WG per frame");
    HIPCHK(attn_bwd(readout_h(L, c.ws), c.io->basis, (const float*)(c.pk + L.k_Q), c.Wf(L.Am), c.Wf(L.dAns), L.da, F, P,
                    L.nq, c.Wf(L.dO), c.Wf(L.dQp), st, 0, 0, (cqm_layout(L) & kCqmDO) != 0));
  }
  tail.reset(new TimerScope(AAA_TIMER_TAIL_BWD, st, 0.0, "bias column sums, query MLP backward, grad unpack"));
  {
    ColSums cs;
    cs.add(c.Wf(L.dY), L.ldy, L.ldy, c.Wf(L.gbhd));
    cs.add(c.Wf(L.dLG), 1024, 1024, c.Wf(L.gblc));
    cs.add(c.Wf(L.dAO), 256, 256, grads + L.poff[A2B]);
    cs.add(c.Wf(L.dH1), 512, 512, grads + L.poff[A0B]);
    cs.add(c.Wf(L.dQp), L.qd, L.qd, c.Wf(L.dQs));
    HIPCHK(colsum_multi(cs, F, st));
  }
  HIPCHK(query_bwd(c.Wf(L.dQs), grads + L.poff[A0B], prm + L.poff[A0W], L.ans_in, L.nq, prm + L.poff[Q2W],
                   prm + L.poff[Q4W], (const float*)(c.pk + L.k_q1), (const float*)(c.pk + L.k_q2), grads + L.poff[Q4W],
                   grads + L.poff[Q4B], grads + L.poff[Q2W], grads + L.poff[Q2B], grads + L.poff[Q0B], st));
  if (ss) HIPCHK(stream_order(ss, st));
  HIPCHK(tail_unpack(L, c.ws, grads, false, st));
  return AAA_OK;
}

template <typename T>
static int head_backward(const BwdCtx& c) {
  const Layout& L = c.L;
  {
    TimerScope tim(AAA_TIMER_MISC, c.st, 0.0, "grad/accumulator memsets, cotangent concat");
    ZeroRanges z{};
    z.add(c.grads, (long)L.ptotal);
    z.add(c.Wf(L.dQs), (long)((L.ws - L.dQs) / 4));
    HIPCHK(prologue<T>(z, 0, nullptr, (T*)nullptr, L.F, L.A, L.ldy, c.io->dlogits, c.io->dvalues, c.Wf(L.dY), c.st));
  }
  return L.sc ? head_backward_stateful(c) : head_backward_zero_state(c);
}

template <typename T>
static int chunk_vision(const BwdCtx& c, int lo, int hi, hipStream_t vs) {
  const Layout& L = c.L;
  const int F1 = (hi - lo) * L.B;
  const size_t f0 = (size_t)lo * L.B;
  const bool on = vbwd_on<T>(L, F1);
  TimerScope tim(AAA_TIMER_VISION_BWD, vs, (double)F1 * vision_bwd_flop(L),
                 on ? "frame-resident conv2 wgrad + dgrad + conv1 wgrad [kernel: k_vision_bwd_frames]"
                    : "conv2 wgrad + dgrad, conv1 wgrad");
  const void* fr = (const char*)c.io->frames + f0 * L.H * L.W * 3 * (L.fu8 ? 1 : 4);
  const bool chunked = L.xpc < L.F;
  return vision_bwd_alone<T>(L, c.pk, fr, c.Wt<T>(L.dY2) + f0 * L.P * 64, c.Wt<T>(L.Y1) + f0 * L.P1 * 32,
                             chunked ? c.Wt<T>(L.Xp) : c.Wt<T>(L.Xp) + f0 * (L.H + 2) * (L.W + 2) * 4,
                             c.Wt<T>(L.dY1) + f0 * L.P1 * 32, nullptr, 0, F1, c.Wf(L.gWp2), c.Wf(L.gWp1),
                             c.grads + L.poff[C0B], vs, chunked ? fr : nullptr, nullptr);
}

template <typename T>
static int batched_dx(const BwdCtx& c, int lo, int hi, hipStream_t s) {
  const Layout& L = c.L;
  const int M = L.B * L.P, rows = (hi - lo) * M;
  const T* dz = c.Wt<T>(L.dZ) + (size_t)lo * M * 512;
  float* gb2 = c.grads + L.poff[C1B];
  TimerScope tim(AAA_TIMER_CORE_DX, s, 2.0 * rows * 64 * 4608, "batched dx (conv2-output grad), K=4608 [kernel: EpiStoreBiasT]");
  const ConvGeo g = ConvGeo{512, 512, 0, L.h, L.w, L.h, L.w, 3, 1, 1, 1}.prep();
  const T* WdT = (const T*)(c.pk + L.k_WdTl);
  const uint32_t zb = (uint32_t)((size_t)rows * 512 * L.esz);
  if constexpr (std::is_same<T, float>::value) {
    EpiStoreBiasT<float> ep{c.Wf(L.dY2) + (size_t)lo * M * 64, 64, 64, rows, gb2};
    using ED = EpiStoreBiasT<float>;
    const int dx6 = f32_split6() ? ab_int("AAA_DX_S6_TILE", 4) : -1;
    if (dx6 == 4) {
      using C6 = GemmCfgS6<64, 128, 32, 2, 2>;
      using LA3 = GRows3B<64, 32, C6::NT>;
      using LBx = GIm2colB<float, 128, 32, C6::NT>;
      HIPCHK((launch_pipe<C6, LA3, LBx, ED, 2>(
          typename LA3::Params{(const __bf16*)(c.pk + L.k_WdT6), 4608, 64, (size_t)64 * 4608},
          typename LBx::Params{dz, g, rows, zb}, ep, 64, rows, 4608, 1, s)));
    } else if (dx6 < 0) {
      if (pipe_batched())
        HIPCHK((step_gemm<CfgFor<T>, true, T, T, ED>(WdT, 4608, 64, dz, g, rows, zb, ep, 64, 4608, s)));
      else
        HIPCHK((step_gemm<CfgFor<T>, false, T, T, ED>(WdT, 4608, 64, dz, g, rows, zb, ep, 64, 4608, s)));
    } else {
#ifdef AAA_ABLATION
      using HF6 = HaloCfgS6<64, 128, 32, 1, 2, 1, 176>;
      switch (dx6) {
        case 6: {
          if (!halo_fits<HF6>(L.h, L.w, 512)) return fail(AAA_E_ARG, "AAA_DX_S6_TILE=6: grid too large");
          const HaloParams hp{WdT, 4608, 64, dz, 512, 0, 512, zb, L.h, L.w, (hi - lo) * L.B, 1};
          HIPCHK((launch_halo<HF6>(hp, ep, s)));
          break;
        }
        case 3: {
          HIPCHK(reorder_cmaj(WdT, 64, 512, 9, 32, (float*)(c.pk + L.k_WdTc), s));
          ConvGeo gc = g;
          gc.cmaj = 32;
          HIPCHK((step_gemm<GemmCfgS6<64, 128, 32, 2, 2>, true, T, T, ED>((const T*)(c.pk + L.k_WdTc), 4608, 64, dz, gc,
                                                                         rows, zb, ep, 64, 4608, s)));
          break;
        }
        case 1:
          HIPCHK((step_gemm<GemmCfgS6<64, 128, 32, 2, 2>, true, T, T, ED>(WdT, 4608, 64, dz, g, rows, zb, ep, 64, 4608, s)));
          break;
        case 5: {
          if (!L.dZ6) return fail(AAA_E_ARG, "AAA_DX_S6_TILE=5 set after the workspace was laid out");
          using C6 = GemmCfgS6<64, 128, 32, 2, 2>;
          using LA3 = GRows3B<64, 32, C6::NT>;
          using LB3 = GIm2colB3<128, 32, C6::NT>;
          __bf16* z6 = (__bf16*)c.Wf(L.dZ6);
          HIPCHK(split_planes(dz, (long)rows * 512, z6, s));
          HIPCHK((launch_pipe<C6, LA3, LB3, ED, 2>(
              typename LA3::Params{(const __bf16*)(c.pk + L.k_WdT6), 4608, 64, (size_t)64 * 4608},
              typename LB3::Params{z6, g, rows, zb / 2, (size_t)rows * 512}, ep, 64, rows, 4608, 1, s)));
          break;
        }
        case 2:
          HIPCHK((step_gemm<GemmCfgS6<64, 64, 64, 2, 2>, true, T, T, ED>(WdT, 4608, 64, dz, g, rows, zb, ep, 64, 4608, s)));
          break;
        default:
          HIPCHK((step_gemm<GemmCfgS6<64, 64, 32, 2, 2>, true, T, T, ED>(WdT, 4608, 64, dz, g, rows, zb, ep, 64, 4608, s)));
      }
#else
      return fail(AAA_E_ARG, "AAA_DX_S6_TILE %d: ablation builds only", dx6);
#endif
    }
  } else {
    EpiStoreBiasT<T> ep{c.Wt<T>(L.dY2) + (size_t)lo * M * 64, 64, 64, rows, gb2};
    using HD = HaloCfg<__bf16, 64, 128, 64, 1, 2, 1, 176>;
    using HW = HaloCfg<__bf16, 64, 512, 32, 1, 4, 1, 576>;
    const HaloParams hp{WdT, 4608, 64, dz, 512, 0, 512, zb, L.h, L.w, (hi - lo) * L.B, 1};
    if (halo_fits<HD>(L.h, L.w, 512) && ab_int("AAA_HALO_DX", 1)) {
// ... 200 lines not shown
  const int M = L.B * L.P;
  const bool vision_here = (phases & AAA_BWD_VISION) != 0;
  hipStream_t ax = aux_stream();
  hipStream_t os = ax ? ax : st;
  const int cs = chunk_steps(L);
  std::unique_ptr<TimerScope> misc(new TimerScope(AAA_TIMER_MISC, st, 0.0, "BPTT state in, last-step gate backward"));
  {
    ZeroRanges z{};
    if (!io->dcT) z.add(c.Wf(L.dC), (long)M * 128);
    z.add(c.Wf(L.rflags), (long)8 * L.B);
    z.add(c.Wf(L.dxb), (long)L.B * 64);
    HIPCHK(prologue<T>(z, 0, nullptr, (T*)nullptr, 0, 0, 1, nullptr, nullptr, nullptr, st));
    if (io->dcT) HIPCHK(hipMemcpyAsync(c.Wf(L.dC), io->dcT, (size_t)M * 128 * 4, hipMemcpyDeviceToDevice, st));
  }
  const int bwd_tile = step_tile((long)(128 / 32) * cdiv(M, 32), "AAA_BPTT_TILE", true, L.dt == AAA_BF16);
  if (bwd_tile < 0) return tile_unknown("AAA_BPTT_TILE");
  BpttChain ch = for_tile<BpttTiles>(bwd_tile, BpttChain{}, [bwd_tile](auto tile) {
    using Tl = decltype(tile);
    return BpttChain{bwd_tile, Tl::split == SplitK::None ? Tl::template Cfg<T>::BJ : kSplitBj, Tl::template pipe<T>(),
                     Tl::split, Tl::dh0, false, nullptr};
  });
  const bool fixk = ch.split == SplitK::SliceFix;
  if (fixk && L.dhs)
    HIPCHK(hipMemsetAsync(c.ws + L.dhs + (size_t)std::max(kBpttSplitMax * 128, 4 * 512) * M * 4, 0, 4096, st));
  ch.g16 = gates_f16(L.dt, M);
  const int fb = frames_bwd(L, ch.g16);
  const bool fb32 = std::is_same<T, float>::value && (!c.reset || f32_split6()) && f32_frames(L) == 8 &&
                    env_int("AAA_F32_FRAMES_BWD", 1);
  ch.part = ch.pipe && !fixk && !fb32 && !c.reset ? c.Wf(L.dZp) : nullptr;
  if (!fb)
    if (const int rc = bptt_last_gates<T>(c, ch)) return rc;
  misc.reset();
  bool dx_fused = false;
  if (fb) {
    if (const int rc = bptt_frames_bf16<T>(c, fb)) return rc;
    dx_fused = true;
  } else if (fb32) {
    if (const int rc = bptt_frames_f32<T>(c, &dx_fused)) return rc;
  }
  int done_hi = L.T;
  auto flush = [&](int ready_lo) -> int {
    while (done_hi - ready_lo >= cs || (ready_lo == 0 && done_hi > 0)) {
      const int lo = std::max(ready_lo, done_hi - cs);
      if (ax) HIPCHK(stream_order(st, ax));
      if (const int rc = core_chunk<T>(c, lo, done_hi, os, dx_fused, vision_here)) return rc;
      done_hi = lo;
    }
    return AAA_OK;
  };
  for (int t = (fb || fb32) ? -1 : L.T - 1; t >= 0; --t) {
    if (const int rc = flush(t)) return rc;
    if (t == 0 && !io->dh0) break;
    if (const int rc = bptt_step<T>(c, ch, t)) return rc;
  }
  if (const int rc = flush(0)) return rc;
  misc.reset(new TimerScope(AAA_TIMER_MISC, st, 0.0, "gate-bias column sums, state grads out, grad unpack"));
  if (fb)
    HIPCHK(colsum<float>(c.Wf(L.dZp), 512, L.T * L.B * fb, 512, c.Wf(L.gbl), st));
  else if (fb32)
    HIPCHK(colsum<float>(c.Wf(L.dZp), 512, L.T * L.B, 512, c.Wf(L.gbl), st));
  else if (ch.part) HIPCHK(colsum<float>(ch.part, 512, L.T * cdiv(M, ch.bj), 512, c.Wf(L.gbl), st));
  else HIPCHK(colsum<T>(c.Wt<T>(L.dZ), 512, L.F * L.P, 512, c.Wf(L.gbl), st));
  if (c.reset)
    HIPCHK(reset_rows(c.reset, L.B, L.P, ResetZeros{}.add(c.Wf(L.dC), 128, 128).add(io->dh0, 128, 128), nullptr, nullptr,
                      0, st));
  if (io->dc0) HIPCHK(hipMemcpyAsync(io->dc0, c.Wf(L.dC), (size_t)M * 128 * 4, hipMemcpyDeviceToDevice, st));
  if (ax) HIPCHK(stream_order(ax, st));
  LstmGrads lg;
  for (int g = 0; g < 4; ++g) {
    lg.wx[g] = c.grads + L.poff[XI_W + 3 * g];
    lg.bx[g] = c.grads + L.poff[XI_B + 3 * g];
    lg.wh[g] = c.grads + L.poff[HI_W + 3 * g];
  }
  if (deferred_unpack) *deferred_unpack = lg;
  else HIPCHK(unpack_lstm(c.Wf(L.gWpl), c.Wf(L.gbl), lg, st));
  return AAA_OK;
}

template <typename T>
static int vision_backward(const BwdCtx& c, int phases, const LstmGrads& core_unpack) {
  const Layout& L = c.L;
  const bool vision_here = (phases & AAA_BWD_CORE) != 0;
  TimerScope tim(AAA_TIMER_VISION_BWD, c.st, vision_here ? 0.0 : (double)L.F * vision_bwd_flop(L),
                 vision_bwd_variant(vbwd_on<T>(L, L.F)));
  if (!vision_here) {
    const int rc = vision_bwd_alone<T>(L, c.pk, c.io->frames, c.Wt<T>(L.dY2), c.Wt<T>(L.Y1), c.Wt<T>(L.Xp),
                                       c.Wt<T>(L.dY1), nullptr, 0, L.F, c.Wf(L.gWp2), c.Wf(L.gWp1),
                                       c.grads + L.poff[C0B], c.st, L.xpc < L.F ? c.io->frames : nullptr, nullptr);
    if (rc) return rc;
  }
  HIPCHK(unpack_cv(vision_here ? c.Wf(L.gWpl) : nullptr, c.Wf(L.gbl), core_unpack, c.Wf(L.gWp2),
                   c.grads + L.poff[C1W], c.Wf(L.gWp1), c.grads + L.poff[C0W], c.st));
  return AAA_OK;
}

template <typename T>
int backward_impl(const Layout& L, const aaa_io* io, int phases, hipStream_t st, const float* reset) {
  TailPrecision tail_prec(std::is_same<T, __bf16>::value && env_int("AAA_TAIL_SPLIT3", 1),
                          std::is_same<T, float>::value && f32_split6());
  const BwdCtx c{L, io, (char*)io->workspace, (const char*)io->packed, io->params, io->grads, st, reset};
  const bool vision = (phases & AAA_BWD_VISION) != 0;
  LstmGrads core_unpack{};
  if (phases & AAA_BWD_HEAD)
    if (const int rc = head_backward<T>(c)) return rc;
  if (phases & AAA_BWD_CORE)
    if (const int rc = core_backward<T>(c, phases, vision ? &core_unpack : nullptr)) return rc;
  if (vision)
    if (const int rc = vision_backward<T>(c, phases, core_unpack)) return rc;
  return AAA_OK;
}

template int lstm_wgrad<float>(const float*, const float*, int, int, int, float*, hipStream_t, bool);
template int lstm_wgrad<__bf16>(const __bf16*, const __bf16*, int, int, int, float*, hipStream_t, bool);
template int vision_bwd<float>(const Layout&, const char*, const float*, const float*, float*, float*, int,
                               float*, float*, float*, hipStream_t, const void*);
template int vision_bwd<__bf16>(const Layout&, const char*, const __bf16*, const __bf16*, __bf16*, __bf16*, int,
                                float*, float*, float*, hipStream_t, const void*);
template int vision_bwd_alone<float>(const Layout&, const char*, const void*, const float*, const float*, float*,
                                     float*, void*, size_t, int, float*, float*, float*, hipStream_t, const void*,
                                     bool*);
template int vision_bwd_alone<__bf16>(const Layout&, const char*, const void*, const __bf16*, const __bf16*, __bf16*,
                                      __bf16*, void*, size_t, int, float*, float*, float*, hipStream_t, const void*,
                                      bool*);
template int backward_impl<float>(const Layout&, const aaa_io*, int, hipStream_t, const float*);
template int backward_impl<__bf16>(const Layout&, const aaa_io*, int, hipStream_t, const float*);

}
```

### towards-interpretable-reinforcement-learning-using-attention-augmented-agents-replication_amd/csrc/rt_components.hip

```cpp
#include "rt.h"

namespace aaa {


struct CellLayout {
  int B, h, w, M, dt, esz;
  size_t k_WpX, k_WpH, k_WdTl, k_bl, k_WpXH, packed;
  size_t XH, Cst, Hs, Gt, dZ, dC, dO, dX, gW, gb, ws;
};

static int cell_layout(const aaa_cell_desc* d, CellLayout& C) {
  if (!d) return fail(AAA_E_ARG, "cell desc is NULL");
  if (d->B < 1 || d->h < 1 || d->w < 1) return fail(AAA_E_ARG, "cell: need B, h, w >= 1");
  if (d->dtype != AAA_F32 && d->dtype != AAA_BF16) return fail(AAA_E_ARG, "cell: bad dtype %d", d->dtype);
  const size_t M = (size_t)d->B * d->h * d->w, e = d->dtype == AAA_BF16 ? 2 : 4;
  if (M * 512 * 4 >= (size_t(1) << 31))
    return fail(AAA_E_ARG, "cell: B*h*w = %zu pixels is above the 2 GiB descriptor range; split the batch", M);
  C.B = d->B; C.h = d->h; C.w = d->w; C.M = (int)M; C.dt = d->dtype; C.esz = (int)e;
  size_t p = 0;
  auto take = [&](size_t bytes) { size_t r = p; p = al256(p + bytes); return r; };
  C.k_WpX = take(512 * 576 * e);
  C.k_WpH = take(512 * 1152 * e);
  C.k_WdTl = take(192 * 4608 * e);
  C.k_bl = take(512 * 4);
// ... 395 lines not shown
    if (p && !aligned16(p)) return fail(AAA_E_ALIGN, "buffers must be 16-byte aligned");
  const Layout& L = C.L;
  char* ws = (char*)workspace;
  auto run = [&](auto tag) -> int {
    using T = decltype(tag);
    int rc = vision_fwd<T, float>(L, L.F, (const char*)packed, cnn_params, frames, (T*)(ws + C.Xp), (T*)(ws + C.Y1),
                                  y2, 64, stream);
    if (rc) return rc;
    if (y1) HIPCHK((cast<T, float>((long)L.F * L.P1 * 32, (const T*)(ws + C.Y1), y1, stream)));
    return AAA_OK;
  };
  return L.dt == AAA_BF16 ? run(__bf16{}) : run(float{});
}

int aaa_vision_cnn_bwd(const aaa_cnn_desc* d, const void* packed, const float* dy2, float* dy1, float* cnn_grads,
                       void* workspace, hipStream_t stream) {
  CnnLayout C;
  int r = cnn_layout(d, C);
  if (r) return r;
  if ((r = check_device())) return r;
  if (!packed || !dy2 || !cnn_grads || !workspace)
    return fail(AAA_E_ARG, "vision_cnn_bwd: packed/dy2/cnn_grads/workspace must be set");
  const void* ptrs[] = {packed, dy2, dy1, cnn_grads, workspace};
  for (const void* p : ptrs)
    if (p && !aligned16(p)) return fail(AAA_E_ALIGN, "buffers must be 16-byte aligned");
  return C.L.dt == AAA_BF16
             ? cnn_bwd_impl<__bf16>(C, (const char*)packed, dy2, dy1, cnn_grads, (char*)workspace, stream)
             : cnn_bwd_impl<float>(C, (const char*)packed, dy2, dy1, cnn_grads, (char*)workspace, stream);
}

size_t aaa_vision_enc_workspace_bytes(const aaa_enc_desc* d) {
  EncLayout E;
  return enc_layout(d, E) ? 0 : E.ws;
}

int aaa_vision_enc_fwd(const aaa_enc_desc* d, const float* cnn_params, const void* packed, const void* frames,
                       void* xp, void* y1, void* out, hipStream_t stream) {
  EncLayout E;
  int r = enc_layout(d, E);
  if (r) return r;
  if (!cnn_params || !packed || !frames || !xp || !y1 || !out)
    return fail(AAA_E_ARG, "vision_enc_fwd: cnn_params/packed/frames/xp/y1/out must be set");
  const void* ptrs[] = {cnn_params, packed, frames, xp, y1, out};
  for (const void* p : ptrs)
    if (!aligned16(p)) return fail(AAA_E_ALIGN, "buffers must be 16-byte aligned");
  if ((r = check_device())) return r;
  const Layout& L = E.L;
  TimerScope tim(AAA_TIMER_VISION_FWD, stream, (double)L.F * vision_fwd_flop(L), "conv1 + conv2 (vision encoder)");
  std::string ran;
  r = vision_fwd<__bf16, __bf16>(L, L.F, (const char*)packed, cnn_params, frames, (__bf16*)xp, (__bf16*)y1,
                                 (__bf16*)out, d->out_ld, stream, true, &ran);
  tim.variant += ": " + ran;
  return r;
}

int aaa_vision_enc_f32_fwd(const aaa_enc_desc* d, const float* cnn_params, const void* packed, const void* frames,
                           float* xp, float* y1, float* out, hipStream_t stream) {
  if (!d) return fail(AAA_E_ARG, "enc desc is NULL");
  if (d->dtype != AAA_F32) return fail(AAA_E_ARG, "vision_enc_f32: fp32 only (dtype %d)", d->dtype);
  if (d->N < 1) return fail(AAA_E_ARG, "vision_enc_f32: need N >= 1");
  if (d->flags & ~AAA_FLAG_FRAMES_U8) return fail(AAA_E_ARG, "vision_enc_f32: flags may hold AAA_FLAG_FRAMES_U8 only");
  if (d->out_ld < 64 || d->out_ld % 8)
    return fail(AAA_E_ARG, "vision_enc_f32: out_ld must be >= 64 and a multiple of 8 (got %d)", d->out_ld);
  const aaa_cfg cfg{d->N, 1, d->H, d->W, 4, 18, d->dtype, d->flags};
  Layout L;
  int r = build_layout(&cfg, L, 1);
  if (r) return r;
  if ((size_t)L.F * L.P * d->out_ld * 4 >= (size_t(1) << 31))
    return fail(AAA_E_ARG, "vision_enc_f32: N*h*w*out_ld is above the 2 GiB descriptor range; split N");
  if (!cnn_params || !packed || !frames || !xp || !y1 || !out)
    return fail(AAA_E_ARG, "vision_enc_f32_fwd: cnn_params/packed/frames/xp/y1/out must be set");
  const void* ptrs[] = {cnn_params, packed, frames, xp, y1, out};
  for (const void* p : ptrs)
    if (!aligned16(p)) return fail(AAA_E_ALIGN, "buffers must be 16-byte aligned");
  if ((r = check_device())) return r;
  TimerScope tim(AAA_TIMER_VISION_FWD, stream, (double)L.F * vision_fwd_flop(L), "conv1 + conv2 (vision encoder)");
  std::string ran;
  r = vision_fwd<float, float>(L, L.F, (const char*)packed, cnn_params, frames, xp, y1, out, d->out_ld, stream, true,
                               &ran);
  tim.variant += ": " + ran;
  return r;
}

int aaa_vision_enc_bwd(const aaa_enc_desc* d, const void* packed, const void* frames, const void* dy2,
                       const void* y1, void* xp, void* dy1, float* cnn_grads, int* fused, void* workspace,
                       hipStream_t stream) {
  EncLayout E;
  int r = enc_layout(d, E);
  if (r) return r;
  if (!packed || !frames || !dy2 || !y1 || !xp || !dy1 || !cnn_grads || !workspace)
    return fail(AAA_E_ARG, "vision_enc_bwd: packed/frames/dy2/y1/xp/dy1/cnn_grads/workspace must be set");
  const void* ptrs[] = {packed, frames, dy2, y1, xp, dy1, cnn_grads, workspace};
  for (const void* p : ptrs)
    if (!aligned16(p)) return fail(AAA_E_ALIGN, "buffers must be 16-byte aligned");
  if ((r = check_device())) return r;
  const Layout& L = E.L;
  char* ws = (char*)workspace;
  float* gW1 = (float*)(ws + E.gW1);
  float* gW2 = (float*)(ws + E.gW2);
  HIPCHK(hipMemsetAsync(cnn_grads, 0, L.poff[XI_W] * 4, stream));
  HIPCHK(hipMemsetAsync(gW1, 0, 32 * 256 * 4, stream));
  HIPCHK(hipMemsetAsync(gW2, 0, 64 * 512 * 4, stream));
  HIPCHK(colsum<__bf16>((const __bf16*)dy2, 64, L.F * L.P, 64, cnn_grads + L.poff[C1B], stream));
  bool on = false;
  {
    TimerScope tim(AAA_TIMER_VISION_BWD, stream, (double)L.F * vision_bwd_flop(L), "");
    r = vision_bwd_alone<__bf16>(L, (const char*)packed, frames, (const __bf16*)dy2, (const __bf16*)y1, (__bf16*)xp,
                                 (__bf16*)dy1, ws + E.part, E.part_bytes, L.F, gW2, gW1, cnn_grads + L.poff[C0B],
                                 stream, nullptr, &on);
    tim.variant = vision_bwd_variant(on);
    if (r) return r;
    HIPCHK(unpack_cv(nullptr, nullptr, LstmGrads{}, gW2, cnn_grads + L.poff[C1W], gW1, cnn_grads + L.poff[C0W], stream));
  }
  if (fused) *fused = on ? 1 : 0;
  return AAA_OK;
}

static int check_attn_args(int F, int h, int w, int nq, int q_stride) {
  if (F < 1 || h < 1 || w < 1) return fail(AAA_E_ARG, "attn: need F, h, w >= 1");
  if (nq != 4 && nq != 8) return fail(AAA_E_ARG, "attn: nq must be 4 or 8 (got %d)", nq);
  if (q_stride != 0 && q_stride != nq * 72) return fail(AAA_E_ARG, "attn: q_stride must be 0 or nq*72");
  if ((size_t)F * h * w * 128 >= (size_t(1) << 31)) return fail(AAA_E_ARG, "attn: F*h*w too large; split F");
  return AAA_OK;
}

static int check_attn(int F, int h, int w, int nq, int q_stride) {
  const int r = check_attn_args(F, h, w, nq, q_stride);
  return r ? r : check_device();
}

static int check_attn_bf16(int F, int h, int w, int nq, int q_stride, int o_ld) {
  const int r = check_attn_args(F, h, w, nq, q_stride);
  if (r) return r;
  if (o_ld < 136 || o_ld % 8)
    return fail(AAA_E_ARG, "attn: bf16 O needs a row pitch o_ld >= 136 and a multiple of 8 (got %d)", o_ld);
  if ((size_t)h * w * o_ld * 2 >= (size_t(1) << 31)) return fail(AAA_E_ARG, "attn: h*w*o_ld too large");
  return AAA_OK;
}

int aaa_attn_fwd(int F, int h, int w, int nq, const float* O, const float* S, const float* Q, int q_stride,
                 const float* prev_reward, const float* prev_action, float* attn, float* answer, hipStream_t stream) {
  int r = check_attn(F, h, w, nq, q_stride);
  if (r) return r;
  if (!O || !S || !Q || !attn || !answer) return fail(AAA_E_ARG, "attn_fwd: O/S/Q/attn/answer must be set");
  if (!aligned16(O) || !aligned16(S)) return fail(AAA_E_ALIGN, "O and S must be 16-byte aligned");
  TimerScope tim(AAA_TIMER_ATTN_FWD, stream, (double)F * attn_fwd_bytes(h * w, nq, 256 * nq + 2), "k_attn_fwd (aaa_attn_fwd)");
  HIPCHK(attn_fwd(o_f32(O), S, Q, nullptr, prev_reward, prev_action, F, h * w, nq, attn, answer, 256 * nq + 2, stream,
                  q_stride));
  return AAA_OK;
}

int aaa_attn_bwd(int F, int h, int w, int nq, const float* O, const float* S, const float* Q, int q_stride,
                 const float* attn, const float* danswer, float* dO, float* dQ, hipStream_t stream) {
  int r = check_attn(F, h, w, nq, q_stride);
  if (r) return r;
  if (!O || !S || !Q || !attn || !danswer || !dO || !dQ)
    return fail(AAA_E_ARG, "attn_bwd: O/S/Q/attn/danswer/dO/dQ must be set");
  if (!aligned16(O) || !aligned16(S) || !aligned16(dO)) return fail(AAA_E_ALIGN, "O, S, dO must be 16-byte aligned");
  TimerScope tim(AAA_TIMER_ATTN_BWD, stream, (double)F * attn_bwd_bytes(h * w, nq), "k_attn_bwd (aaa_attn_bwd)");
  HIPCHK(attn_bwd(o_f32(O), S, Q, attn, danswer, 256 * nq + 2, F, h * w, nq, dO, dQ, stream, q_stride, 1));
  return AAA_OK;
}

int aaa_attn_fwd_bf16(int F, int h, int w, int nq, const void* O, int o_ld, const float* S, const float* Q,
                      int q_stride, float* sq_scratch, const float* prev_reward, const float* prev_action,
                      float* attn, float* answer, hipStream_t stream) {
// ... 50 lines not shown
```

### towards-interpretable-reinforcement-learning-using-attention-augmented-agents-replication_amd/csrc/rt_core.hip

```cpp
#include "rt.h"

namespace aaa {

thread_local std::string g_err;
thread_local bool g_tail3 = false, g_tail6 = false;

int fail(int code, const char* fmt, ...) {
  char buf[512];
  va_list ap;
  va_start(ap, fmt);
  vsnprintf(buf, sizeof buf, fmt, ap);
  va_end(ap);
  g_err = buf;
  return code;
}

static int check_ranges(Layout& L, int min_frames);

int build_layout(const aaa_cfg* c, Layout& L, int min_frames) {
  if (!c) return fail(AAA_E_ARG, "cfg is NULL");
  if (c->B < 1 || c->T < 1) return fail(AAA_E_ARG, "B and T must be >= 1 (B=%d T=%d)", c->B, c->T);
  if (c->nq != 4 && c->nq != 8) return fail(AAA_E_ARG, "nq must be 4 or 8 (got %d)", c->nq);
  if (c->A < 1 || c->A > 256) return fail(AAA_E_ARG, "A out of range (%d)", c->A);
  if (c->dtype != AAA_F32 && c->dtype != AAA_BF16) return fail(AAA_E_ARG, "bad dtype %d", c->dtype);
  if (c->flags & ~(AAA_FLAG_STATEFUL_CORE | AAA_FLAG_FRAMES_U8 | AAA_FLAG_DEFER_STRANDED)) return fail(AAA_E_ARG, "unknown flags 0x%x", c->flags);
  L.sc = (c->flags & AAA_FLAG_STATEFUL_CORE) != 0;
  L.fu8 = (c->flags & AAA_FLAG_FRAMES_U8) != 0;
  L.B = c->B; L.T = c->T; L.F = c->B * c->T; L.H = c->H; L.W = c->W;
  L.H1 = conv_out(c->H, 8, 4, 1); L.W1 = conv_out(c->W, 8, 4, 1);
  L.h = conv_out(L.H1, 4, 2, 2); L.w = conv_out(L.W1, 4, 2, 2);
  if (L.H1 < 1 || L.W1 < 1 || L.h < 1 || L.w < 1) return fail(AAA_E_ARG, "frame %dx%d too small", c->H, c->W);
  L.P1 = L.H1 * L.W1; L.P = L.h * L.w;
  L.nq = c->nq; L.A = c->A; L.dt = c->dtype; L.esz = c->dtype == AAA_BF16 ? 2 : 4;
  L.qd = 72 * L.nq; L.da = (L.sc ? 256 : 184) * L.nq; L.ans_in = 256 * L.nq + 2;
  L.ans_ld = (L.ans_in + 7) / 8 * 8;
  L.ldy = (2 * L.A + 3) / 4 * 4;
  const size_t shp[NPARAM] = {
      32 * 3 * 64, 32, 64 * 32 * 16, 64,
      128 * 64 * 9, 128, 128 * 128 * 9, 128 * 64 * 9, 128, 128 * 128 * 9,
      128 * 64 * 9, 128, 128 * 128 * 9, 128 * 64 * 9, 128, 128 * 128 * 9,
      128 * 256, 128, (size_t)L.qd * 128, (size_t)L.qd, (size_t)L.qd * L.qd, (size_t)L.qd,
      512 * (size_t)L.ans_in, 512, 256 * 512, 256,
      1024 * 256, 1024 * 256, 1024, 1024,
      (size_t)L.A * 256, (size_t)L.A, (size_t)L.A * 256, (size_t)L.A};
  size_t o = 0;
  for (int i = 0; i < NPARAM; ++i) { L.poff[i] = o; L.psz[i] = shp[i]; o += shp[i]; }
  L.ptotal = o;
  size_t p = 0;
  auto take = [&](size_t bytes) { size_t r = p; p = al256(p + bytes); return r; };
  const size_t e = L.esz;
  L.k_Wp1 = take(32 * 256 * e);
  L.k_Wp2 = take(64 * 512 * e);
  L.k_WdT2 = take(4 * 32 * 256 * e);
  L.k_W1s = take(e == 4 ? kVfW1 : 0);
  L.k_W2s = take(e == 4 ? kVfW2 : 0);
  L.k_WpX = take(512 * 576 * e);
  L.k_WpH = take(512 * 1152 * e);
  L.k_WpXH = take(512 * 1728 * e);
  L.k_Wfr = take(e == 2 ? (size_t)16 * kRecKSP * 64 * 16 : 0);
  L.k_WdTl = take(192 * 4608 * e);
  L.k_WdTc = take(e == 4 ? 64 * 4608 * 4 : 0);
  L.k_WdT6 = take(e == 4 ? 3 * 64 * 4608 * 2 : 0);
  L.k_Wbf = take(e == 2 ? (size_t)6 * kBwKSP * 64 * 16 : 0);
  L.k_Wf32 = take(e == 4 ? (size_t)16 * kF32QP * 64 * 16 : 0);
  L.k_Wb32 = take(e == 4 ? (size_t)8 * kB32QP * 4 * 64 * 16 : 0);
  L.k_Wf6 = take(e == 4 ? (size_t)16 * kF32QP * 64 * 24 : 0);
  L.k_Wf6p = take(e == 4 ? (size_t)16 * kF32PP * 3 * 64 * 16 : 0);
  L.k_Wb6 = take(e == 4 ? (size_t)8 * kB32QP * 4 * 64 * 24 : 0);
  L.k_Wx6 = take(e == 4 ? (size_t)8 * kB32QP * 2 * 64 * 24 : 0);
  L.k_Wb6p = take(e == 4 ? (size_t)8 * kB32PP * 4 * 3 * 64 * 16 : 0);
  L.k_Wx6p = take(e == 4 ? (size_t)8 * kB32PP * 2 * 3 * 64 * 16 : 0);
  L.k_bl = take(512 * 4);
  L.k_W1p = take(512 * (size_t)L.ans_ld * 4);
  L.k_Wihp = take(1024 * 256 * 4);
  L.k_blc = take(1024 * 4);
  L.k_Whd = take((size_t)L.ldy * 256 * 4);
  L.k_bhd = take((size_t)L.ldy * 4);
  L.k_Wihhp = take(L.sc ? 1024 * 512 * 4 : 0);
  L.k_q1 = take(128 * 4);
  L.k_q2 = take((size_t)L.qd * 4);
  L.k_Q = take((size_t)L.qd * 4);
  L.packed = p;
  p = 0;
  const size_t F = L.F, P = L.P, M = (size_t)L.B * L.P;
  const int xc = ab_int("AAA_XP_CHUNK", 0);
  L.xpc = xc > 0 ? (int)std::min<size_t>(F, (size_t)std::max(64, xc)) : (int)F;
  L.Xp = take((size_t)L.xpc * (L.H + 2) * (L.W + 2) * 4 * e);
  L.Y1 = take(F * L.P1 * 32 * e);
  L.XH = take((size_t)(L.T + 1) * M * 192 * e);
  L.Hs = take(e == 4 ? F * P * 128 * 4 : 0);
  L.Cst = take((size_t)(L.T + 1) * M * 128 * 4);
  L.Gt = take(F * P * 512 * 4);
  L.SQ = take(P * L.nq * 4);
  L.Am = take(F * P * L.nq * 4);
  L.ans = take(F * L.ans_ld * 4);
  L.hid1 = take(F * 512 * 4);
  L.AO = take(F * 256 * 4);
  L.LG = take(F * 1024 * 4);
  L.LC = take(F * 256 * 4);
  L.LH = take(F * 256 * 4);
  L.dY = take(F * L.ldy * 4);
  L.dLG = take(F * 1024 * 4);
  L.dAO = take(F * 256 * 4);
  L.dH1 = take(F * 512 * 4);
  L.dAns = take(F * L.da * 4);
  L.dO = take(F * P * 128 * 4);
  L.dQp = take(F * L.qd * 4);
  L.dC = take(M * 128 * 4);
  L.dZ = take(F * P * 512 * e);
  L.dZ6 = take(e == 4 && ab_int("AAA_DX_S6_TILE", 4) == 5 ? F * P * 512 * 6 : 0);
  const size_t zp_rows = std::max({(M + 31) / 32, 2 * (size_t)L.B,
                                   L.esz == 4 && bptt_splitk_fits(M) ? (M + kSplitBj - 1) / kSplitBj : 0});
  L.dZp = take((size_t)L.T * zp_rows * 512 * 4);
  L.dY2 = take(F * P * 64 * e);
  L.dY1 = take(F * L.P1 * 32 * e);
  L.dxb = take((size_t)L.B * 64 * 4);
  L.rflags = take((size_t)8 * L.B * 4);
  L.xpart = take(L.esz == 4 && rec_fits(L.h, L.w) ? b32_xpart_floats(L.B) * 4 : 0);
  L.dhs = L.esz == 4 && bptt_splitk_fits(M) ? take((size_t)std::max(kBpttSplitMax * 128, 4 * 512) * M * 4 + 4096) : 0;
  {
    const size_t sc = L.sc ? 1 : 0, B = L.B;
    L.CH = take(sc * (L.T + 1) * B * 256 * 4);
    L.CC = take(sc * (L.T + 1) * B * 256 * 4);
    L.AOX = take(sc * F * 512 * 4);
    L.Qf = take(sc * F * L.qd * 4);
    L.q1s = take(sc * F * 128 * 4);
    L.q2s = take(sc * F * L.qd * 4);
    L.dAOX = take(sc * F * 512 * 4);
    L.dQf = take(sc * F * L.qd * 4);
    L.dq2s = take(sc * F * L.qd * 4);
    L.dq1s = take(sc * F * 128 * 4);
    L.dhc = take(sc * B * 256 * 4);
    L.dcc = take(sc * B * 256 * 4);
  }
  L.dQs = take((size_t)L.qd * 4);
  L.gWp1 = take(32 * 256 * 4);
  L.gWp2 = take(64 * 512 * 4);
  L.gWpl = take(512 * 1728 * 4);
  L.gbl = take(512 * 4);
  L.gW1p = take(512 * (size_t)L.ans_ld * 4);
  L.gWihp = take(1024 * 256 * 4);
  L.gblc = take(1024 * 4);
  L.gWhd = take((size_t)L.ldy * 256 * 4);
  L.gbhd = take((size_t)L.ldy * 4);
  L.gWihhp = take(L.sc ? 1024 * 512 * 4 : 0);
  L.ws = p;
  return check_ranges(L, min_frames > 0 ? min_frames : L.B);
}

static int check_ranges(Layout& L, int min_frames) {
  const size_t lim = size_t(1) << 31, F = (size_t)L.F, e = (size_t)L.esz;
  const size_t per_frame = std::max({(size_t)(L.H + 2) * (L.W + 2) * 4 * e,
                                     (size_t)L.P1 * 32 * e,
                                     (size_t)L.P * 512 * e,
                                     (size_t)L.P * 192 * e,
                                     (size_t)L.P * 64 * e,
                                     (size_t)L.H * L.W * 3 * 4});
  const size_t fc = (lim - 1) / per_frame;
  if (fc < (size_t)min_frames)
    return fail(AAA_E_ARG, "B=%d %dx%d: one step's operands (%zu bytes) exceed the 2 GiB a buffer descriptor "
                "addresses; split the batch (data-parallel ranks or several calls)", L.B, L.H, L.W,
                per_frame * min_frames);
  L.fchunk = (int)std::min(fc, F);
  const size_t elems[] = {F * L.P * 512, F * L.P * 128, F * (size_t)L.ans_ld, F * 1024, F * (size_t)L.P1 * 32,
// ... 202 lines not shown
```

### towards-interpretable-reinforcement-learning-using-attention-augmented-agents-replication_amd/csrc/rt_forward.hip

```cpp
#include "rt.h"

namespace aaa {

template <typename T>
int pack_impl(const Layout& L, const float* prm, char* pk, hipStream_t st) {
  PackAll<T> a;
  a.c1w = prm + L.poff[C0W];
  a.c2w = prm + L.poff[C1W];
  a.Wp1 = (T*)(pk + L.k_Wp1); a.Wp2 = (T*)(pk + L.k_Wp2); a.WdT2 = (T*)(pk + L.k_WdT2);
  if constexpr (std::is_same<T, float>::value) {
    a.W1s = (__bf16*)(pk + L.k_W1s); a.W2s = (__bf16*)(pk + L.k_W2s);
  }
  for (int g = 0; g < 4; ++g) {
    a.lstm.wx[g] = prm + L.poff[XI_W + 3 * g];
    a.lstm.bx[g] = prm + L.poff[XI_B + 3 * g];
    a.lstm.wh[g] = prm + L.poff[HI_W + 3 * g];
  }
  a.WpX = (T*)(pk + L.k_WpX); a.WpH = (T*)(pk + L.k_WpH); a.WdT = (T*)(pk + L.k_WdTl);
  a.WpXH = (T*)(pk + L.k_WpXH); a.bl = (float*)(pk + L.k_bl);
  F32Pack& fp = a.f32;
  fp.a0w = prm + L.poff[A0W]; fp.wih = prm + L.poff[WIH]; fp.bih = prm + L.poff[BIH]; fp.bhh = prm + L.poff[BHH];
  fp.pw = prm + L.poff[PW]; fp.vw = prm + L.poff[VW]; fp.pb = prm + L.poff[PB]; fp.vb = prm + L.poff[VB];
  fp.W1p = (float*)(pk + L.k_W1p); fp.Wihp = (float*)(pk + L.k_Wihp); fp.blc = (float*)(pk + L.k_blc);
  fp.Whd = (float*)(pk + L.k_Whd); fp.bhd = (float*)(pk + L.k_bhd);
  fp.ans_in = L.ans_in; fp.ans_ld = L.ans_ld; fp.A = L.A; fp.ldy = L.ldy;
  if (L.sc) {
    fp.whh = prm + L.poff[WHH];
    fp.Wihhp = (float*)(pk + L.k_Wihhp);
  }
  HIPCHK(pack_all<T>(a, st));
  if constexpr (!std::is_same<T, float>::value) {
    HIPCHK(pack_wfrag((const __bf16*)(pk + L.k_WpXH), (__bf16*)(pk + L.k_Wfr), st));
    HIPCHK(pack_wbfrag((const __bf16*)(pk + L.k_WdTl), (__bf16*)(pk + L.k_Wbf), st));
  } else {
    HIPCHK(pack_frag_f32(FragPack{(const float*)(pk + L.k_WpXH), (const float*)(pk + L.k_WdTl), (float*)(pk + L.k_Wf32),
                                  (u32x2*)(pk + L.k_Wf6), (u32x4*)(pk + L.k_Wf6p), (float*)(pk + L.k_Wb32),
                                  (u32x2*)(pk + L.k_Wb6), (u32x2*)(pk + L.k_Wx6), (u32x4*)(pk + L.k_Wb6p),
                                  (u32x4*)(pk + L.k_Wx6p), (__bf16*)(pk + L.k_WdT6)},
                         st));
  }
  HIPCHK(query_pack(prm + L.poff[Q0B], prm + L.poff[Q2W], prm + L.poff[Q2B], prm + L.poff[Q4W], prm + L.poff[Q4B], L.nq,
                    (float*)(pk + L.k_q1), (float*)(pk + L.k_q2), (float*)(pk + L.k_Q), st));
  return AAA_OK;
}

template <typename T, typename OT>
static int vision_fwd_chunk(const Layout& L, int F, const char* pk, const float* prm, const void* frames, T* Xp, T* Y1,
                      OT* out, int out_ld, hipStream_t st, bool xp_full, std::string* ran) {
  using C = CfgFor<T>;
  constexpr int NT = C::NT;
  const int P = L.P;
  bool banded = false;
  if constexpr (std::is_same<T, __bf16>::value) {
    if (band_fits(L.H, L.W, L.H1, L.W1) && env_int("AAA_VIS_BAND", 1)) {
      const VisBandParams bp{frames, (const __bf16*)(pk + L.k_Wp1), prm + L.poff[C0B], xp_full ? Xp : nullptr, Y1, F,
                             L.H, L.W, L.H1, L.W1};
      HIPCHK(L.fu8 ? vision_conv1_band<uint8_t>(bp, st) : vision_conv1_band<float>(bp, st));
      banded = true;
    }
  }
  if (!banded) {
    const size_t fb = (size_t)L.H * L.W * 3 * (L.fu8 ? 1 : 4), xb = (size_t)(L.H + 2) * (L.W + 2) * 4;
    const int step = xp_full ? F : L.xpc;
    for (int s0 = 0; s0 < F; s0 += step) {
      const int n = std::min(step, F - s0);
      const char* fr = (const char*)frames + (size_t)s0 * fb;
      T* xp = xp_full ? Xp + (size_t)s0 * xb : Xp;
      if (L.fu8) HIPCHK((frames_rgbx<T, uint8_t>(n, L.H, L.W, (const uint8_t*)fr, xp, st)));
      else HIPCHK((frames_rgbx<T, float>(n, L.H, L.W, (const float*)fr, xp, st)));
      constexpr int BKc = std::is_same<T, float>::value ? 32 : 64;
      EpiStoreT<T> ep{Y1 + (size_t)s0 * L.P1 * 32, 32, 32, n * L.P1, prm + L.poff[C0B], 0};
      auto conv1 = [&](auto cfg) -> int {
        using CP = decltype(cfg);
        using PA = GRowsB<T, CP::BI, CP::BK, CP::NT>;
        using PB = GIm2colB<T, CP::BJ, CP::BK, CP::NT>;
        HIPCHK((launch_pipe<CP, PA, PB, EpiStoreT<T>, 2>(
            typename PA::Params{(const T*)(pk + L.k_Wp1), 256, 32},
            typename PB::Params{xp, ConvGeo{4, 4, 0, L.H + 2, L.W + 2, L.H1, L.W1, 8, 4, 0, 0}.prep(), n * L.P1,
                                (uint32_t)((size_t)n * xb * L.esz)},
            ep, 32, n * L.P1, 256, 1, st)));
        return AAA_OK;
      };
      const int c1t = ab_int("AAA_CONV1_TILE", 0);
      int rc;
      if constexpr (std::is_same<T, float>::value) {
        if (f32_split6()) rc = L.fu8 && ab_int("AAA_CONV1_BEXACT", 1) ? conv1(GemmCfgS6BX<32, 128, BKc, 1, 4>{})
                                                                      : conv1(GemmCfgS6<32, 128, BKc, 1, 4>{});
        else rc = c1t == 1 ? conv1(GemmCfg<T, 32, 256, BKc, 1, 4>{}) : conv1(GemmCfg<T, 32, 128, BKc, 1, 4>{});
      } else {
        rc = c1t == 1 ? conv1(GemmCfg<T, 32, 256, BKc, 1, 4>{}) : conv1(GemmCfg<T, 32, 128, BKc, 1, 4>{});
      }
      if (rc) return rc;
    }
  }
// ... 367 lines not shown
```

### towards-interpretable-reinforcement-learning-using-attention-augmented-agents-replication_amd/runtime.py

```python
from __future__ import annotations

import ctypes

import torch

from . import _native as N


class UnrollRunner:
    def __init__(self, B: int, T: int, H: int, W: int, nq: int = 4, A: int = 18,
                 dtype: str = "fp32", device=None, stateful_core: bool = False, frames_u8: bool = False,
                 defer_stranded: bool = False):
        if dtype not in ("fp32", "bf16"):
            raise ValueError(f"dtype must be 'fp32' or 'bf16', got {dtype!r}")
        self.lib = N.load()
        self.device = torch.device(device if device is not None else "cuda")
        if self.device.type != "cuda":
            raise RuntimeError("aaa: the HIP path needs a ROCm GPU tensor device (no CPU fallback)")
        self.stateful_core = bool(stateful_core)
        self.frames_u8 = bool(frames_u8)
        self.cfg = N.Cfg(B, T, H, W, nq, A, N.BF16 if dtype == "bf16" else N.F32,
                         (N.FLAG_STATEFUL_CORE if stateful_core else 0) | (N.FLAG_FRAMES_U8 if frames_u8 else 0)
                         | (N.FLAG_DEFER_STRANDED if defer_stranded else 0))
        self.B, self.T, self.H, self.W, self.nq, self.A, self.dtype = B, T, H, W, nq, A, dtype
# ... 273 lines not shown
        self.desc = N.EncDesc(N_, H, W, N.BF16, N.FLAG_FRAMES_U8 if frames_u8 else 0, out_ld)
        self.cnn = N.CnnDesc(N_, H, W, N.BF16)
        self.pk_bytes = self.lib.aaa_vision_cnn_packed_bytes(ctypes.byref(self.cnn))
        self.ws_bytes = self.lib.aaa_vision_enc_workspace_bytes(ctypes.byref(self.desc))
        if not self.pk_bytes or not self.ws_bytes:
            N.check(-1, "vision_enc layout")

    def pack(self, cnn_flat):
        packed = torch.empty(self.pk_bytes, dtype=torch.uint8, device=self.device)
        N.check(self.lib.aaa_vision_cnn_pack(ctypes.byref(self.cnn), N.ptr(cnn_flat), N.ptr(packed),
                                             N.stream_ptr(self.device)), "vision_cnn_pack")
        return packed

    def _frames(self, frames):
        want = torch.uint8 if self.u8 else torch.float32
        if frames.dtype != want or tuple(frames.shape) != (self.N, self.H, self.W, 3):
            raise ValueError(f"frames must be {want} of shape {(self.N, self.H, self.W, 3)}")
        return frames.to(self.device).contiguous()

    def forward(self, cnn_flat, packed, frames):
        dev, bf = self.device, torch.bfloat16
        frames = self._frames(frames)
        xp = torch.full((self.N, self.H + 2, self.W + 2, 4), float("nan"), dtype=bf, device=dev)
        y1 = torch.full((self.N, self.H1, self.W1, 32), float("nan"), dtype=bf, device=dev)
        out = torch.full((self.N, self.h * self.w, self.out_ld), self.SENTINEL, dtype=torch.int16, device=dev).view(bf)
        N.check(self.lib.aaa_vision_enc_fwd(ctypes.byref(self.desc), N.ptr(cnn_flat), N.ptr(packed), N.ptr(frames),
                                            N.ptr(xp), N.ptr(y1), N.ptr(out), N.stream_ptr(dev)), "vision_enc_fwd")
        return xp, y1, out

    def backward(self, packed, frames, dy2, y1, xp):
        dev, bf = self.device, torch.bfloat16
        frames = self._frames(frames)
        if dy2.dtype != bf or tuple(dy2.shape) != (self.N, self.h * self.w, 64):
            raise ValueError("dy2 must be bfloat16 (N, h*w, 64)")
        dy2 = dy2.to(dev).contiguous()
        grads = torch.empty(32 * 3 * 64 + 32 + 64 * 32 * 16 + 64, device=dev)
        dy1 = torch.full((self.N, self.H1, self.W1, 32), float("nan"), dtype=bf, device=dev)
        ws = torch.empty(self.ws_bytes, dtype=torch.uint8, device=dev)
        fused = ctypes.c_int(-1)
        N.check(self.lib.aaa_vision_enc_bwd(ctypes.byref(self.desc), N.ptr(packed), N.ptr(frames), N.ptr(dy2),
                                            N.ptr(y1), N.ptr(xp), N.ptr(dy1), N.ptr(grads), ctypes.byref(fused),
                                            N.ptr(ws), N.stream_ptr(dev)), "vision_enc_bwd")
        return grads, (None if fused.value else dy1), bool(fused.value)


class EncF32Runner:

    SENTINEL = 0x7A5B7A5B

    def __init__(self, N_: int, H: int, W: int, out_ld: int = 192, frames_u8: bool = True, device=None):
        self.lib = N.load()
        self.device = torch.device(device if device is not None else "cuda")
        if self.device.type != "cuda":
            raise RuntimeError("aaa: the HIP path needs a ROCm GPU tensor device (no CPU fallback)")
        self.N, self.H, self.W, self.out_ld, self.u8 = N_, H, W, out_ld, frames_u8
        self.h, self.w = N.grid(H, W)
        self.H1, self.W1 = (H + 2 - 8) // 4 + 1, (W + 2 - 8) // 4 + 1
        self.desc = N.EncDesc(N_, H, W, N.F32, N.FLAG_FRAMES_U8 if frames_u8 else 0, out_ld)
        self.cnn = N.CnnDesc(N_, H, W, N.F32)
        self.pk_bytes = self.lib.aaa_vision_cnn_packed_bytes(ctypes.byref(self.cnn))
        if not self.pk_bytes:
            N.check(-1, "vision_enc_f32 layout")

    def pack(self, cnn_flat):
        packed = torch.empty(self.pk_bytes, dtype=torch.uint8, device=self.device)
        N.check(self.lib.aaa_vision_cnn_pack(ctypes.byref(self.cnn), N.ptr(cnn_flat), N.ptr(packed),
                                             N.stream_ptr(self.device)), "vision_cnn_pack")
        return packed

    def forward(self, cnn_flat, packed, frames):
        dev = self.device
        want = torch.uint8 if self.u8 else torch.float32
        if frames.dtype != want or tuple(frames.shape) != (self.N, self.H, self.W, 3):
            raise ValueError(f"frames must be {want} of shape {(self.N, self.H, self.W, 3)}")
        frames = frames.to(dev).contiguous()
        xp = torch.full((self.N, self.H + 2, self.W + 2, 4), float("nan"), device=dev)
        y1 = torch.full((self.N, self.H1, self.W1, 32), float("nan"), device=dev)
        out = torch.full((self.N, self.h * self.w, self.out_ld), self.SENTINEL, dtype=torch.int32,
                         device=dev).view(torch.float32)
        N.check(self.lib.aaa_vision_enc_f32_fwd(ctypes.byref(self.desc), N.ptr(cnn_flat), N.ptr(packed),
                                                N.ptr(frames), N.ptr(xp), N.ptr(y1), N.ptr(out), N.stream_ptr(dev)),
                "vision_enc_f32_fwd")
        return xp, y1, out


class ActorRunner:

    def __init__(self, B: int, H: int, W: int, nq: int = 4, A: int = 18, device=None, frames_u8: bool = True,
                 stateful_core: bool = False):
        self.lib = N.load()
        self.device = torch.device(device if device is not None else "cuda")
        if self.device.type != "cuda":
            raise RuntimeError("aaa: the HIP path needs a ROCm GPU tensor device (no CPU fallback)")
        self.B, self.H, self.W, self.nq, self.A = B, H, W, nq, A
        self.frames_u8 = bool(frames_u8)
        self.stateful_core = bool(stateful_core)
        self.cfg = N.Cfg(B, 1, H, W, nq, A, N.F32, (N.FLAG_FRAMES_U8 if frames_u8 else 0)
                         | (N.FLAG_STATEFUL_CORE if stateful_core else 0))
        self.h, self.w = N.grid(H, W)
        self.P = self.h * self.w
        self.n_params, self.offsets, self.sizes = N.param_layout(self.cfg)
        query = self.lib.aaa_actor_core_workspace_bytes if stateful_core else self.lib.aaa_actor_workspace_bytes
        self.ws_bytes = query(ctypes.byref(self.cfg))
        self.pk_bytes = self.lib.aaa_packed_bytes(ctypes.byref(self.cfg))
        if not self.ws_bytes or not self.pk_bytes:
            N.check(-1, "actor layout")

    def new_workspace(self):
        return torch.empty(self.ws_bytes, dtype=torch.uint8, device=self.device)

    def new_packed(self):
        return torch.empty(self.pk_bytes, dtype=torch.uint8, device=self.device)

    def state_shape(self):
        return (self.B, self.h, self.w, 128)

    def pack(self, flat_params, packed):
        assert flat_params.dtype == torch.float32 and flat_params.is_contiguous()
        assert flat_params.numel() == self.n_params, (flat_params.numel(), self.n_params)
        N.check(self.lib.aaa_pack_weights(ctypes.byref(self.cfg), N.ptr(flat_params), N.ptr(packed),
                                          N.stream_ptr(self.device)), "pack_weights")

    def step(self, flat_params, packed, basis, frames, workspace, h, c, logits, values, attn=None,
             prev_reward=None, prev_action=None, seed: int = 0, counter=None, actions=None, logp=None,
             dlogp=None, gates=None, h_out=None, c_out=None, core_h=None, core_c=None, core_h_out=None,
             core_c_out=None, query=None):
        exp = (self.B, self.H, self.W, 3)
        dt = torch.uint8 if self.frames_u8 else torch.float32
        if tuple(frames.shape[-4:]) != exp or frames.numel() != self.B * self.H * self.W * 3 or \
                frames.dtype != dt or not frames.is_contiguous():
            raise ValueError(f"frames must be contiguous {dt} {exp}, got {tuple(frames.shape)} {frames.dtype}")
        for name, t in (("h", h), ("c", c)):
            if tuple(t.shape) != self.state_shape() or t.dtype != torch.float32 or not t.is_contiguous():
                raise ValueError(f"{name} must be contiguous fp32 {self.state_shape()}")
        io = N.ActorIO()
        for k, v in dict(params=flat_params, packed=packed, basis=basis, frames=frames, prev_reward=prev_reward,
                         prev_action=prev_action, h=h, c=c, logits=logits, values=values, attn=attn,
                         workspace=workspace, counter=counter, actions=actions, logp=logp,
                         dlogp_dlogits=dlogp, gates=gates, h_out=h_out, c_out=c_out).items():
            setattr(io, k, None if v is None else v.data_ptr())
        io.seed = int(seed) & (2**64 - 1)
        core = dict(core_h=core_h, core_c=core_c, core_h_out=core_h_out, core_c_out=core_c_out)
        if not self.stateful_core:
            if query is not None or any(v is not None for v in core.values()):
                raise ValueError("core_h / core_c / query belong to a stateful_core runner")
            N.check(self.lib.aaa_actor_step(ctypes.byref(self.cfg), ctypes.byref(io), N.stream_ptr(self.device)),
                    "actor_step")
            return
        if core_h is None or core_c is None:
            raise ValueError("a stateful_core runner needs core_h and core_c")
        for name, t in core.items():
            if t is not None and (tuple(t.shape) != (self.B, 256) or t.dtype != torch.float32 or not t.is_contiguous()):
                raise ValueError(f"{name} must be contiguous fp32 {(self.B, 256)}")
        if query is not None and (tuple(query.shape) != (self.B, self.nq, 72) or query.dtype != torch.float32
                                  or not query.is_contiguous()):
            raise ValueError(f"query must be contiguous fp32 {(self.B, self.nq, 72)}")
        cio = N.ActorCoreIO()
        for k, v in dict(core, query=query).items():
            setattr(cio, k, None if v is None else v.data_ptr())
        N.check(self.lib.aaa_actor_step_core(ctypes.byref(self.cfg), ctypes.byref(io), ctypes.byref(cio),
                                             N.stream_ptr(self.device)), "actor_step_core")
```

Before: 237,900 frames/s.

## Add frame-resident fused fp32 vision backward kernel using split-bf16 MFMA

Adds a fp32 path for the frame-resident vision backward. One kernel computes conv2 wgrad, conv2 dgrad and conv1 wgrad from the resident frames, using split-bf16 weight packs with MFMA. The per-group partials are then reduced. It also packs a split copy of WdT2 and exposes a standalone encoder backward API. The aim is to replace the separate fp32 conv2 wgrad/dgrad/conv1 wgrad kernels and their intermediate traffic, at the cost of a new complex kernel whose split-bf16 accuracy is the main risk. It is gated on u8 frames, the split6 mode and size fits.

```diff
diff --git a/include/aaa.h b/include/aaa.h
--- a/include/aaa.h
+++ b/include/aaa.h
@@ -277,6 +277,10 @@
                        hipStream_t stream);
 int aaa_vision_enc_f32_fwd(const aaa_enc_desc* d, const float* cnn_params, const void* packed, const void* frames,
                            float* xp, float* y1, float* out, hipStream_t stream);
+size_t aaa_vision_enc_f32_workspace_bytes(const aaa_enc_desc* d);
+int aaa_vision_enc_f32_bwd(const aaa_enc_desc* d, const void* packed, const void* frames, const float* dy2,
+                           const float* y1, float* xp, float* dy1, float* cnn_grads, int* fused, int max_groups,
+                           void* workspace, hipStream_t stream);
 
 int aaa_attn_fwd(int F, int h, int w, int nq, const float* O, const float* S, const float* Q, int q_stride,
                  const float* prev_reward, const float* prev_action, float* attn, float* answer, hipStream_t stream);
diff --git a/towards-interpretable-reinforcement-learning-using-attention-augmented-agents-replication_amd/_native.py b/towards-interpretable-reinforcement-learning-using-attention-augmented-agents-replication_amd/_native.py
--- a/towards-interpretable-reinforcement-learning-using-attention-augmented-agents-replication_amd/_native.py
+++ b/towards-interpretable-reinforcement-learning-using-attention-augmented-agents-replication_amd/_native.py
@@ -30,6 +30,7 @@
     "aaa_forward_resets", "aaa_backward_resets",
     "aaa_vision_enc_f32_fwd",
     "aaa_grad_norm_scratch_bytes", "aaa_grad_norm", "aaa_grad_scale", "aaa_adam_step_clipped",
+    "aaa_vision_enc_f32_workspace_bytes", "aaa_vision_enc_f32_bwd",
 )
 TIMER_FWD_STEP, TIMER_BPTT_STEP, TIMER_CORE_WGRAD, TIMER_ATTN_FWD, TIMER_ATTN_BWD = 0, 1, 2, 3, 4
 TIMER_PACK, TIMER_VISION_FWD, TIMER_TAIL_FWD, TIMER_TAIL_BWD, TIMER_CORE_DX, TIMER_VISION_BWD, TIMER_MISC = range(5, 12)
@@ -183,6 +184,8 @@
             "aaa_vision_enc_fwd": (I, [ctypes.POINTER(EncDesc), P, P, P, P, P, P, P]),
             "aaa_vision_enc_bwd": (I, [ctypes.POINTER(EncDesc), P, P, P, P, P, P, P, ctypes.POINTER(I), P, P]),
             "aaa_vision_enc_f32_fwd": (I, [ctypes.POINTER(EncDesc), P, P, P, P, P, P, P]),
+            "aaa_vision_enc_f32_workspace_bytes": (S, [ctypes.POINTER(EncDesc)]),
+            "aaa_vision_enc_f32_bwd": (I, [ctypes.POINTER(EncDesc), P, P, P, P, P, P, P, ctypes.POINTER(I), I, P, P]),
             "aaa_attn_fwd": (I, [I, I, I, I, P, P, P, I, P, P, P, P, P]),
             "aaa_attn_bwd": (I, [I, I, I, I, P, P, P, I, P, P, P, P, P]),
             "aaa_attn_fwd_bf16": (I, [I, I, I, I, P, I, P, P, I, P, P, P, P, P, P]),
diff --git a/towards-interpretable-reinforcement-learning-using-attention-augmented-agents-replication_amd/csrc/misc.h b/towards-interpretable-reinforcement-learning-using-attention-augmented-agents-replication_amd/csrc/misc.h
--- a/towards-interpretable-reinforcement-learning-using-attention-augmented-agents-replication_amd/csrc/misc.h
+++ b/towards-interpretable-reinforcement-learning-using-attention-augmented-agents-replication_amd/csrc/misc.h
@@ -38,9 +38,11 @@
   float* bl;
   F32Pack f32;
   __bf16 *W1s = nullptr, *W2s = nullptr;
+  __bf16* WdT2s = nullptr;
 };
 template <typename T> hipError_t pack_all(const PackAll<T>& a, hipStream_t st);
 hipError_t pack_vis_split(const float* c1w, const float* c2w, __bf16* W1s, __bf16* W2s, hipStream_t st);
+hipError_t pack_wdt2_split(const float* WdT2, __bf16* WdT2s, hipStream_t st);
 
 hipError_t query_pack(const float* b0, const float* W2, const float* b2, const float* W4, const float* b4, int nq,
                       float* q1, float* q2, float* Q, hipStream_t st);
diff --git a/towards-interpretable-reinforcement-learning-using-attention-augmented-agents-replication_amd/csrc/misc.hip b/towards-interpretable-reinforcement-learning-using-attention-augmented-agents-replication_amd/csrc/misc.hip
--- a/towards-interpretable-reinforcement-learning-using-attention-augmented-agents-replication_amd/csrc/misc.hip
+++ b/towards-interpretable-reinforcement-learning-using-attention-augmented-agents-replication_amd/csrc/misc.hip
@@ -899,6 +899,11 @@
     }
   }
 }
+__global__ void k_pack_wdt2_split(const float* __restrict__ WdT2, __bf16* WdT2s) {
+  const int tot = 4 * 32 * 256;
+  for (int idx = blockIdx.x * blockDim.x + threadIdx.x; idx < tot; idx += gridDim.x * blockDim.x)
+    vis_split_el(WdT2[idx], idx >> 8, idx & 255, 16, WdT2s);
+}
 
 template <typename T>
 __global__ void k_pack_all(PackAll<T> a) {
@@ -914,7 +919,11 @@
       if constexpr (std::is_same<T, float>::value)
         if (a.W2s) vis_split_el(a.Wp2[idx - n1], (idx - n1) >> 9, (idx - n1) & 511, 32, a.W2s);
     }
-    else if (idx < n3) pack_conv2_classes_el(idx - n2, a.c2w, a.WdT2);
+    else if (idx < n3) {
+      pack_conv2_classes_el(idx - n2, a.c2w, a.WdT2);
+      if constexpr (std::is_same<T, float>::value)
+        if (a.WdT2s) vis_split_el(a.WdT2[idx - n2], (idx - n2) >> 8, (idx - n2) & 255, 16, a.WdT2s);
+    }
     else if (idx < n4) pack_lstm_el(idx - n3, a.lstm, a.WpX, a.WpH, a.bl, a.WdT, a.WpXH);
     else pack_f32_el(idx - n4, a.f32);
   }
@@ -1368,6 +1377,10 @@
   hipLaunchKernelGGL(k_pack_all<T>, dim3(nblk(n)), dim3(256), 0, st, a);
   return hipGetLastError();
 }
+hipError_t pack_wdt2_split(const float* WdT2, __bf16* WdT2s, hipStream_t st) {
+  hipLaunchKernelGGL(k_pack_wdt2_split, dim3(nblk(4L * 32 * 256)), dim3(256), 0, st, WdT2, WdT2s);
+  return hipGetLastError();
+}
 hipError_t pack_vis_split(const float* c1w, const float* c2w, __bf16* W1s, __bf16* W2s, hipStream_t st) {
   hipLaunchKernelGGL(k_pack_vis_split, dim3(nblk(32L * 256 + 64 * 512)), dim3(256), 0, st, c1w, c2w, W1s, W2s);
   return hipGetLastError();
diff --git a/towards-interpretable-reinforcement-learning-using-attention-augmented-agents-replication_amd/csrc/rt.h b/towards-interpretable-reinforcement-learning-using-attention-augmented-agents-replication_amd/csrc/rt.h
--- a/towards-interpretable-reinforcement-learning-using-attention-augmented-agents-replication_amd/csrc/rt.h
+++ b/towards-interpretable-reinforcement-learning-using-attention-augmented-agents-replication_amd/csrc/rt.h
@@ -26,6 +26,7 @@
 #include "vision.h"
 #include "vision_f32.h"
 #include "vision_bwd.h"
+#include "vision_bwd_f32.h"
 #include "misc.h"
 #include "optim.h"
 #include "actor.h"
@@ -67,7 +68,7 @@
   int xpc;
   int qd, da, ans_in, ans_ld, ldy;
   size_t poff[NPARAM], psz[NPARAM], ptotal;
-  size_t k_Wp1, k_Wp2, k_WdT2, k_W1s, k_W2s, k_WpX, k_WpH, k_WpXH, k_Wfr, k_Wbf, k_Wf32, k_Wb32, k_Wf6, k_Wf6p, k_Wb6, k_Wx6, k_Wb6p, k_Wx6p, k_WdTl, k_WdTc, k_WdT6, k_bl, k_Wihhp, k_q1, k_q2, k_Q, k_W1p, k_Wihp, k_blc, k_Whd, k_bhd, packed;
+  size_t k_Wp1, k_Wp2, k_WdT2, k_W1s, k_W2s, k_WpX, k_WpH, k_WpXH, k_Wfr, k_Wbf, k_Wf32, k_Wb32, k_Wf6, k_Wf6p, k_Wb6, k_Wx6, k_Wb6p, k_Wx6p, k_WdTl, k_WdTc, k_WdT6, k_bl, k_Wihhp, k_q1, k_q2, k_Q, k_W1p, k_Wihp, k_blc, k_Whd, k_bhd, k_WdT2s, packed;
   size_t Xp, Y1, XH, Hs, Cst, Gt, SQ, Am, ans, hid1, AO, LG, LC, LH;
   size_t dY, dLG, dAO, dH1, dAns, dO, dQp, dQs, dC, dZ, dZp, dY2, dY1, dxb, rflags, xpart, dhs, dZ6;
   size_t gWp1, gWp2, gWpl, gbl, gW1p, gWihp, gblc, gWhd, gbhd, ws;
@@ -445,11 +446,12 @@
 template <typename T>
 int vision_bwd(const Layout& L, const char* pk, const T* dy2, const T* y1, T* xp, T* dy1, int F, float* gW2,
                float* gW1, float* gb1, hipStream_t s, const void* frames = nullptr);
-const char* vision_bwd_variant(bool fused);
+const char* vision_bwd_variant(bool fused, bool f32 = false, bool unpack = true);
 template <typename T>
 int vision_bwd_alone(const Layout& L, const char* pk, const void* frames, const T* dy2, const T* y1, T* xp, T* dy1,
                      void* part, size_t part_bytes, int F, float* gW2, float* gW1, float* gb1, hipStream_t st,
-                     const void* xp_frames, bool* fused);
+                     const void* xp_frames, bool* fused, int max_groups = 0, float* dy1_out = nullptr,
+                     const void* wdt2s = nullptr);
 template <typename T>
 int backward_impl(const Layout& L, const aaa_io* io, int phases, hipStream_t st, const float* reset = nullptr);
 
diff --git a/towards-interpretable-reinforcement-learning-using-attention-augmented-agents-replication_amd/csrc/rt_backward.hip b/towards-interpretable-reinforcement-learning-using-attention-augmented-agents-replication_amd/csrc/rt_backward.hip
--- a/towards-interpretable-reinforcement-learning-using-attention-augmented-agents-replication_amd/csrc/rt_backward.hip
+++ b/towards-interpretable-reinforcement-learning-using-attention-augmented-agents-replication_amd/csrc/rt_backward.hip
@@ -344,9 +344,16 @@
   return AAA_OK;
 }
 
+static size_t vbwd_f32_room(const Layout& L, int F, size_t part_bytes) {
+  return part_bytes ? part_bytes : (size_t)(L.xpc < L.F ? L.xpc : F) * (L.H + 2) * (L.W + 2) * 4 * 4;
+}
 template <typename T>
 static bool vbwd_on(const Layout& L, int F, size_t part_bytes = 0) {
-  if constexpr (!std::is_same<T, __bf16>::value) {
+  if constexpr (std::is_same<T, float>::value) {
+    return f32_split6() && L.fu8 && vbwd_f32_fits(L.H, L.W, L.H1, L.W1, L.h, L.w) && env_int("AAA_VIS_FRAMES", 1) &&
+           env_int("AAA_VIS_BWD_FRAMES", 1) && F >= env_int("AAA_VBWD_MINF", 1) * device_cus() &&
+           vbwd_f32_groups(F, device_cus(), vbwd_f32_room(L, F, part_bytes)) >= 1;
+  } else if constexpr (!std::is_same<T, __bf16>::value) {
     (void)L; (void)F; (void)part_bytes;
     return false;
   } else {
@@ -358,9 +365,16 @@
 }
 template <typename T>
 static int vbwd_run(const Layout& L, const char* pk, const void* frames, int f0, int F, const T* dy2, const T* y1,
-                    T* dy1, float* gW2, float* gW1, float* gb1, hipStream_t s) {
-  if constexpr (!std::is_same<T, __bf16>::value) {
-    return fail(AAA_E_ARG, "the frame-resident vision backward is bf16 only");
+                    T* dy1, float* gW2, float* gW1, float* gb1, hipStream_t s, size_t part_bytes = 0,
+                    int max_groups = 0, float* dy1_out = nullptr, const void* wdt2s = nullptr) {
+  if constexpr (std::is_same<T, float>::value) {
+    VisBwdF32Params vp{(const char*)frames + (size_t)f0 * L.H * L.W * 3, dy2, y1,
+                       (const bf16x8*)(wdt2s ? wdt2s : pk + L.k_WdT2s),
+                       dy1, dy1_out, F, L.H, L.W, L.H1, L.W1, L.h, L.w};
+    HIPCHK(vision_bwd_frames_f32(vp, vbwd_f32_groups(F, device_cus(), part_bytes, max_groups), gW2, gW1, gb1, s));
+    return AAA_OK;
+  } else if constexpr (!std::is_same<T, __bf16>::value) {
+    return fail(AAA_E_ARG, "the frame-resident vision backward is bf16 / fp32 only");
   } else {
     VisBwdParams vp{(const char*)frames + (size_t)f0 * L.H * L.W * 3 * (L.fu8 ? 1 : 4), dy2, y1,
                     (const __bf16*)(pk + L.k_WdT2), (float*)dy1, F, L.H, L.W, L.H1, L.W1, L.h, L.w};
@@ -369,17 +383,26 @@
   }
 }
 
-const char* vision_bwd_variant(bool fused) {
-  return fused ? "frame-resident conv2 wgrad + dgrad + conv1 wgrad [kernel: k_vision_bwd_frames], grad unpack"
-               : "conv2 wgrad + dgrad, conv1 wgrad, grad unpack";
+const char* vision_bwd_variant(bool fused, bool f32, bool unpack) {
+  static const char* const v[3][2] = {
+      {"conv2 wgrad + dgrad, conv1 wgrad", "conv2 wgrad + dgrad, conv1 wgrad, grad unpack"},
+      {"frame-resident conv2 wgrad + dgrad + conv1 wgrad [kernel: k_vision_bwd_frames]",
+       "frame-resident conv2 wgrad + dgrad + conv1 wgrad [kernel: k_vision_bwd_frames], grad unpack"},
+      {"frame-resident conv2 wgrad + dgrad + conv1 wgrad [kernel: k_vision_bwd_f32]",
+       "frame-resident conv2 wgrad + dgrad + conv1 wgrad [kernel: k_vision_bwd_f32], grad unpack"}};
+  return v[!fused ? 0 : f32 ? 2 : 1][unpack];
 }
 template <typename T>
 int vision_bwd_alone(const Layout& L, const char* pk, const void* frames, const T* dy2, const T* y1, T* xp, T* dy1,
                      void* part, size_t part_bytes, int F, float* gW2, float* gW1, float* gb1, hipStream_t st,
-                     const void* xp_frames, bool* fused) {
+                     const void* xp_frames, bool* fused, int max_groups, float* dy1_out, const void* wdt2s) {
   const bool on = vbwd_on<T>(L, F, part_bytes);
   if (fused) *fused = on;
-  if (on) return vbwd_run<T>(L, pk, frames, 0, F, dy2, y1, part ? (T*)part : dy1, gW2, gW1, gb1, st);
+  if (on) {
+    constexpr bool f32 = std::is_same<T, float>::value;
+    return vbwd_run<T>(L, pk, frames, 0, F, dy2, y1, part ? (T*)part : f32 ? xp : dy1, gW2, gW1, gb1, st,
+                       f32 ? vbwd_f32_room(L, F, part_bytes) : 0, max_groups, dy1_out, wdt2s);
+  }
   const int rc = vision_bwd<T>(L, pk, dy2, y1, xp, dy1, F, gW2, gW1, gb1, st, xp_frames);
   if (rc) return rc;
   if (std::is_same<T, float>::value && !ab_int("AAA_CONV2_DGRAD_RING", 1))
@@ -559,8 +582,7 @@
   const size_t f0 = (size_t)lo * L.B;
   const bool on = vbwd_on<T>(L, F1);
   TimerScope tim(AAA_TIMER_VISION_BWD, vs, (double)F1 * vision_bwd_flop(L),
-                 on ? "frame-resident conv2 wgrad + dgrad + conv1 wgrad [kernel: k_vision_bwd_frames]"
-                    : "conv2 wgrad + dgrad, conv1 wgrad");
+                 vision_bwd_variant(on, std::is_same<T, float>::value, false));
   const void* fr = (const char*)c.io->frames + f0 * L.H * L.W * 3 * (L.fu8 ? 1 : 4);
   const bool chunked = L.xpc < L.F;
   return vision_bwd_alone<T>(L, c.pk, fr, c.Wt<T>(L.dY2) + f0 * L.P * 64, c.Wt<T>(L.Y1) + f0 * L.P1 * 32,
@@ -927,7 +949,7 @@
   const Layout& L = c.L;
   const bool vision_here = (phases & AAA_BWD_CORE) != 0;
   TimerScope tim(AAA_TIMER_VISION_BWD, c.st, vision_here ? 0.0 : (double)L.F * vision_bwd_flop(L),
-                 vision_bwd_variant(vbwd_on<T>(L, L.F)));
+                 vision_bwd_variant(vbwd_on<T>(L, L.F), std::is_same<T, float>::value));
   if (!vision_here) {
     const int rc = vision_bwd_alone<T>(L, c.pk, c.io->frames, c.Wt<T>(L.dY2), c.Wt<T>(L.Y1), c.Wt<T>(L.Xp),
                                        c.Wt<T>(L.dY1), nullptr, 0, L.F, c.Wf(L.gWp2), c.Wf(L.gWp1),
@@ -963,10 +985,10 @@
                                 float*, float*, float*, hipStream_t, const void*);
 template int vision_bwd_alone<float>(const Layout&, const char*, const void*, const float*, const float*, float*,
                                      float*, void*, size_t, int, float*, float*, float*, hipStream_t, const void*,
-                                     bool*);
+                                     bool*, int, float*, const void*);
 template int vision_bwd_alone<__bf16>(const Layout&, const char*, const void*, const __bf16*, const __bf16*, __bf16*,
                                       __bf16*, void*, size_t, int, float*, float*, float*, hipStream_t, const void*,
-                                      bool*);
+                                      bool*, int, float*, const void*);
 template int backward_impl<float>(const Layout&, const aaa_io*, int, hipStream_t, const float*);
 template int backward_impl<__bf16>(const Layout&, const aaa_io*, int, hipStream_t, const float*);
 
diff --git a/towards-interpretable-reinforcement-learning-using-attention-augmented-agents-replication_amd/csrc/rt_components.hip b/towards-interpretable-reinforcement-learning-using-attention-augmented-agents-replication_amd/csrc/rt_components.hip
--- a/towards-interpretable-reinforcement-learning-using-attention-augmented-agents-replication_amd/csrc/rt_components.hip
+++ b/towards-interpretable-reinforcement-learning-using-attention-augmented-agents-replication_amd/csrc/rt_components.hip
@@ -501,6 +501,71 @@
   return r;
 }
 
+struct EncF32Layout {
+  Layout L;
+  size_t gW1, gW2, part, part_bytes, dY1, Ws, ws;
+};
+static int enc_f32_layout(const aaa_enc_desc* d, EncF32Layout& E) {
+  if (!d) return fail(AAA_E_ARG, "enc desc is NULL");
+  if (d->dtype != AAA_F32) return fail(AAA_E_ARG, "vision_enc_f32: fp32 only (dtype %d)", d->dtype);
+  if (d->N < 1) return fail(AAA_E_ARG, "vision_enc_f32: need N >= 1");
+  if (d->flags & ~AAA_FLAG_FRAMES_U8) return fail(AAA_E_ARG, "vision_enc_f32: flags may hold AAA_FLAG_FRAMES_U8 only");
+  const aaa_cfg cfg{d->N, 1, d->H, d->W, 4, 18, d->dtype, d->flags};
+  const int r = build_layout(&cfg, E.L, 1);
+  if (r) return r;
+  size_t p = 0;
+  auto take = [&](size_t bytes) { size_t q = p; p = al256(p + bytes); return q; };
+  E.gW1 = take(32 * 256 * 4);
+  E.gW2 = take(64 * 512 * 4);
+  E.part_bytes = (size_t)E.L.F * kVbPart * 4;
+  E.part = take(E.part_bytes);
+  E.dY1 = take((size_t)E.L.F * E.L.P1 * 32 * 4);
+  E.Ws = take(kVqWs);
+  E.ws = p;
+  return AAA_OK;
+}
+
+size_t aaa_vision_enc_f32_workspace_bytes(const aaa_enc_desc* d) {
+  EncF32Layout E;
+  return enc_f32_layout(d, E) ? 0 : E.ws;
+}
+
+int aaa_vision_enc_f32_bwd(const aaa_enc_desc* d, const void* packed, const void* frames, const float* dy2,
+                           const float* y1, float* xp, float* dy1, float* cnn_grads, int* fused, int max_groups,
+                           void* workspace, hipStream_t stream) {
+  EncF32Layout E;
+  int r = enc_f32_layout(d, E);
+  if (r) return r;
+  if (max_groups < 0) return fail(AAA_E_ARG, "vision_enc_f32_bwd: max_groups must be >= 0");
+  if (!packed || !frames || !dy2 || !y1 || !xp || !cnn_grads || !workspace)
+    return fail(AAA_E_ARG, "vision_enc_f32_bwd: packed/frames/dy2/y1/xp/cnn_grads/workspace must be set");
+  const void* ptrs[] = {packed, frames, dy2, y1, xp, dy1, cnn_grads, workspace};
+  for (const void* p : ptrs)
+    if (!aligned16(p)) return fail(AAA_E_ALIGN, "buffers must be 16-byte aligned");
+  if ((r = check_device())) return r;
+  const Layout& L = E.L;
+  char* ws = (char*)workspace;
+  float* gW1 = (float*)(ws + E.gW1);
+  float* gW2 = (float*)(ws + E.gW2);
+  HIPCHK(hipMemsetAsync(cnn_grads, 0, L.poff[XI_W] * 4, stream));
+  HIPCHK(hipMemsetAsync(gW1, 0, 32 * 256 * 4, stream));
+  HIPCHK(hipMemsetAsync(gW2, 0, 64 * 512 * 4, stream));
+  HIPCHK(colsum<float>(dy2, 64, L.F * L.P, 64, cnn_grads + L.poff[C1B], stream));
+  HIPCHK(pack_wdt2_split((const float*)((const char*)packed + L.k_WdT2), (__bf16*)(ws + E.Ws), stream));
+  bool on = false;
+  {
+    TimerScope tim(AAA_TIMER_VISION_BWD, stream, (double)L.F * vision_bwd_flop(L), "");
+    r = vision_bwd_alone<float>(L, (const char*)packed, frames, dy2, y1, xp, dy1 ? dy1 : (float*)(ws + E.dY1),
+                                ws + E.part, E.part_bytes, L.F, gW2, gW1, cnn_grads + L.poff[C0B], stream, nullptr,
+                                &on, max_groups, dy1, ws + E.Ws);
+    tim.variant = vision_bwd_variant(on, true);
+    if (r) return r;
+    HIPCHK(unpack_cv(nullptr, nullptr, LstmGrads{}, gW2, cnn_grads + L.poff[C1W], gW1, cnn_grads + L.poff[C0W], stream));
+  }
+  if (fused) *fused = on ? 1 : 0;
+  return AAA_OK;
+}
+
 int aaa_vision_enc_bwd(const aaa_enc_desc* d, const void* packed, const void* frames, const void* dy2,
                        const void* y1, void* xp, void* dy1, float* cnn_grads, int* fused, void* workspace,
                        hipStream_t stream) {
diff --git a/towards-interpretable-reinforcement-learning-using-attention-augmented-agents-replication_amd/csrc/rt_core.hip b/towards-interpretable-reinforcement-learning-using-attention-augmented-agents-replication_amd/csrc/rt_core.hip
--- a/towards-interpretable-reinforcement-learning-using-attention-augmented-agents-replication_amd/csrc/rt_core.hip
+++ b/towards-interpretable-reinforcement-learning-using-attention-augmented-agents-replication_amd/csrc/rt_core.hip
@@ -80,6 +80,7 @@
   L.k_q1 = take(128 * 4);
   L.k_q2 = take((size_t)L.qd * 4);
   L.k_Q = take((size_t)L.qd * 4);
+  L.k_WdT2s = take(e == 4 ? kVqWs : 0);
   L.packed = p;
   p = 0;
   const size_t F = L.F, P = L.P, M = (size_t)L.B * L.P;
diff --git a/towards-interpretable-reinforcement-learning-using-attention-augmented-agents-replication_amd/csrc/rt_forward.hip b/towards-interpretable-reinforcement-learning-using-attention-augmented-agents-replication_amd/csrc/rt_forward.hip
--- a/towards-interpretable-reinforcement-learning-using-attention-augmented-agents-replication_amd/csrc/rt_forward.hip
+++ b/towards-interpretable-reinforcement-learning-using-attention-augmented-agents-replication_amd/csrc/rt_forward.hip
@@ -10,6 +10,7 @@
   a.Wp1 = (T*)(pk + L.k_Wp1); a.Wp2 = (T*)(pk + L.k_Wp2); a.WdT2 = (T*)(pk + L.k_WdT2);
   if constexpr (std::is_same<T, float>::value) {
     a.W1s = (__bf16*)(pk + L.k_W1s); a.W2s = (__bf16*)(pk + L.k_W2s);
+    a.WdT2s = (__bf16*)(pk + L.k_WdT2s);
   }
   for (int g = 0; g < 4; ++g) {
     a.lstm.wx[g] = prm + L.poff[XI_W + 3 * g];
diff --git a/towards-interpretable-reinforcement-learning-using-attention-augmented-agents-replication_amd/csrc/vision_bwd_f32.h b/towards-interpretable-reinforcement-learning-using-attention-augmented-agents-replication_amd/csrc/vision_bwd_f32.h
--- /dev/null
+++ b/towards-interpretable-reinforcement-learning-using-attention-augmented-agents-replication_amd/csrc/vision_bwd_f32.h
@@ -0,0 +1,384 @@
+#pragma once
+#include "vision_bwd.h"
+
+namespace aaa {
+
+constexpr int kVqD = 0;
+constexpr int kVqY = 3 * kVbDB;
+constexpr int kVqLds = kVqY + 3 * kVbYB;
+constexpr int kVqT = kVqLds - 3 * kVbTB;
+constexpr int kVqX = 0;
+constexpr int kVqWs = 4 * 16 * 3 * 64 * 16;
+static_assert(kVqLds <= 160 * 1024, "phase 1: three dY2 and three Y1 planes");
+static_assert(kVqT >= kVqD + 3 * kVbDB, "phase 2: the dY1 planes clear of the dY2 planes the dgrad reads");
+static_assert(kVqX + kVisXB <= kVqT, "phase 3: the RGBx image clear of the dY1 planes");
+static_assert(kVqT % 16 == 0 && kVqY % 16 == 0, "16-B LDS accesses");
+static_assert(kVbK1 % 16 == 0 && kVbDN * 64 == 8 * 256 * 4 && kVbK1 * 32 <= 13 * 256 * 4, "register prefetch slots");
+static_assert(256 * 16 * 4 <= kVqLds, "bias-sum scratch");
+
+struct VisBwdF32Params {
+  const void* frames;
+  const float* dY2;
+  const float* Y1;
+  const bf16x8* Ws;
+  float* part;
+  float* dy1;
+  int F, H, W, H1, W1, h, w;
+};
+
+inline bool vbwd_f32_fits(int H, int W, int H1, int W1, int h, int w) {
+  const int Ha = (H1 + 1) / 2, Wa = (W1 + 1) / 2;
+  return vis_fits(H, W, H1, W1, h, w) && h * w <= kVbDN - 1 && H1 * W1 <= kVbK1 && Ha * Wa <= 128 && w < 128 &&
+         (H1 + 4) * (W1 + 4) * 64 <= kVbYB && Ha <= h && Wa <= w && W1 >= 8;
+}
+
+__device__ __forceinline__ void vq_commit4(unsigned char* base, int plane, const f32x4& v) {
+  bf16x4 ph, pm, pl;
+#pragma unroll
+  for (int e = 0; e < 4; ++e) {
+    ph[e] = (__bf16)v[e];
+    const float r = v[e] - (float)ph[e];
+    pm[e] = (__bf16)r;
+    pl[e] = (__bf16)(r - (float)pm[e]);
+  }
+  *reinterpret_cast<bf16x4*>(base) = ph;
+  *reinterpret_cast<bf16x4*>(base + plane) = pm;
+  *reinterpret_cast<bf16x4*>(base + 2 * plane) = pl;
+}
+
+template <bool DY1>
+__global__ void __launch_bounds__(256) __attribute__((amdgpu_waves_per_eu(1, 1))) k_vision_bwd_f32(VisBwdF32Params p) {
+  __shared__ __attribute__((aligned(16))) unsigned char lds[kVqLds];
+  unsigned char* const dpl = lds + kVqD;
+  unsigned char* const ypl = lds + kVqY;
+  unsigned char* const tpl = lds + kVqT;
+  unsigned char* const xim = lds + kVqX;
+  const int tid = (int)threadIdx.x, lane = tid & 63;
+  const int wave = __builtin_amdgcn_readfirstlane(tid >> 6);
+  const int r32 = lane & 31, hh = lane >> 5;
+  const int Wp = p.W + 2, W1p = p.W1 + 4, P = p.h * p.w, P1 = p.H1 * p.W1;
+  const int Ha = (p.H1 + 1) / 2, Wa = (p.W1 + 1) / 2, NA = Ha * Wa;
+  const int G4 = p.H * p.W / 4;
+  const int KS1 = (P1 + 15) / 16;
+
+  {
+    u32x4* z = reinterpret_cast<u32x4*>(lds);
+    for (int i = tid; i < kVqLds / 16; i += 256) z[i] = u32x4{0u, 0u, 0u, 0u};
+  }
+
+  f32x4 rd[8], ry[13];
+  uint32_t raw[kVisNG][3];
+  auto fetch = [&](int f, int tid) {
+    const f32x4* d = reinterpret_cast<const f32x4*>(p.dY2 + (size_t)f * P * 64);
+#pragma unroll
+    for (int k = 0; k < 8; ++k) rd[k] = d[min(tid + 256 * k, P * 16 - 1)];
+    const f32x4* y = reinterpret_cast<const f32x4*>(p.Y1 + (size_t)f * P1 * 32);
+#pragma unroll
+    for (int k = 0; k < 13; ++k) ry[k] = y[min(tid + 256 * k, P1 * 8 - 1)];
+    const uint32_t* src =
+        reinterpret_cast<const uint32_t*>(reinterpret_cast<const uint8_t*>(p.frames) + (size_t)f * p.H * p.W * 3);
+    int two = 2;
+    asm volatile("" : "+s"(two));
+#pragma unroll
+    for (int i = 0; i < kVisNG; ++i) {
+      const int g = min(tid + 256 * i, G4 - 1);
+      const uint2 v = *reinterpret_cast<const uint2*>(src + (size_t)g * 3);
+      raw[i][0] = v.x;
+      raw[i][1] = v.y;
+      raw[i][2] = src[(size_t)g * 3 + two];
+    }
+  };
+  auto commit = [&](int tid) {
+#pragma unroll
+    for (int k = 0; k < 8; ++k) {
+      const int i = tid + 256 * k, pix = i >> 4, ch = (i & 15) * 4;
+      const f32x4 v = pix < P ? rd[k] : f32x4{0.f, 0.f, 0.f, 0.f};
+      vq_commit4(dpl + vb_dofs(pix, ch), kVbDB, v);
+    }
+#pragma unroll
+    for (int k = 0; k < 13; ++k) {
+      const int i = tid + 256 * k, p1 = i >> 3, ch = (i & 7) * 4;
+      if (p1 < P1) {
+        const int y = p1 / p.W1, x = p1 - y * p.W1;
+        vq_commit4(ypl + ((y + 2) * W1p + x + 2) * 64 + ch * 2, kVbYB, ry[k]);
+      }
+    }
+    for (int i = tid; i < (p.H1 + 4) * W1p; i += 256) {
+      const int y = i / W1p, x = i - y * W1p;
+      if (y < 2 || y >= p.H1 + 2 || x < 2 || x >= p.W1 + 2) {
+#pragma unroll
+        for (int q = 0; q < 3; ++q) {
+          u32x4* z = reinterpret_cast<u32x4*>(ypl + q * kVbYB + i * 64);
+#pragma unroll
+          for (int c = 0; c < 4; ++c) z[c] = u32x4{0u, 0u, 0u, 0u};
+        }
+      }
+    }
+  };
+  auto build = [&](int tid) {
+    for (int i = tid; i < 2 * Wp + 2 * p.H; i += 256) {
+      const int px = i < 2 * Wp ? (i < Wp ? i : (p.H + 1) * Wp + i - Wp)
+                                : (1 + ((i - 2 * Wp) >> 1)) * Wp + ((i & 1) ? Wp - 1 : 0);
+      *reinterpret_cast<uint2*>(xim + px * 8) = uint2{0u, 0u};
+    }
+#pragma unroll
+    for (int i = 0; i < kVisNG; ++i) {
+      const int g = tid + 256 * i;
+      if (g < G4) {
+        const int pix = 4 * g, y = pix / p.W, x = pix - y * p.W;
+        unsigned char* d = xim + ((y + 1) * Wp + x + 1) * 8;
+#pragma unroll
+        for (int j = 0; j < 4; ++j) {
+          float v[3];
+#pragma unroll
+          for (int c = 0; c < 3; ++c) {
+            const int e = 3 * j + c;
+            v[c] = (float)((raw[i][e >> 2] >> (8 * (e & 3))) & 255u);
+          }
+          *reinterpret_cast<bf16x4*>(d + j * 8) = bf16x4{(__bf16)v[0], (__bf16)v[1], (__bf16)v[2], (__bf16)0.f};
+        }
+      }
+    }
+  };
+
+  const int rw16 = (65536 + p.w - 1) / p.w;
+  auto ypo = [&](int pix) {
+    pix = pix < P ? pix : 0;
+    const int y2 = (pix * rw16) >> 16, x2 = pix - y2 * p.w;
+    return (2 * y2 * W1p + 2 * x2) * 64;
+  };
+
+  f32x16 acc2[2][4], acc1[2];
+#pragma unroll
+  for (int e = 0; e < 16; ++e) {
+#pragma unroll
+    for (int r = 0; r < 2; ++r)
+#pragma unroll
+      for (int j = 0; j < 4; ++j) acc2[r][j][e] = 0.f;
+    acc1[0][e] = acc1[1][e] = 0.f;
+  }
+  float bsum[16];
+#pragma unroll
+  for (int i = 0; i < 16; ++i) bsum[i] = 0.f;
+  const int py = wave >> 1, px = wave & 1;
+
+  int f = blockIdx.x;
+  if (f < p.F) fetch(f, tid);
+  barrier_lds();
+  for (; f < p.F; f += gridDim.x) {
+    auto launder = [&](int l = 0) {
+      asm volatile("" : "+v"(l));
+      return l;
+    };
+    commit(tid + launder());
+    barrier_lds();
+
+    {
+      const int wl = lane + launder(), r32 = wl & 31, hh = wl >> 5, tq = (wl & 15) >> 2, tp = wl & 3;
+      bf16x8 a2[2][2][3], b2[2][4][3];
+      auto ld2 = [&](int s, int i) {
+        const int k0 = 16 * s + 8 * hh + tq;
+        if (i < 6) {
+          const int rb = i / 3, q = i % 3, o0 = 32 * rb + (r32 & 16) + 4 * tp;
+          a2[s & 1][rb][q] = vb_tr(dpl + q * kVbDB, vb_dofs(k0, o0), vb_dofs(k0 + 4, o0));
+        } else {
+          const int j = (i - 6) / 3, q = (i - 6) % 3;
+          const int tap = 4 * wave + j, ky = tap >> 2, kx = tap & 3;
+          const int off = (ky * W1p + kx) * 64 + ((r32 & 16) + 4 * tp) * 2;
+          b2[s & 1][j][q] = vb_tr(ypl + q * kVbYB, ypo(k0) + off, ypo(k0 + 4) + off);
+        }
+      };
+#pragma unroll
+      for (int i = 0; i < 18; ++i) ld2(0, i);
+#pragma unroll
+      for (int s = 0; s < 8; ++s) {
+        constexpr int qa[6] = {2, 0, 1, 1, 0, 0}, qb[6] = {0, 2, 1, 0, 1, 0};
+#pragma unroll
+        for (int g = 0; g < 6; ++g) {
+          if (s + 1 < 8) {
+#pragma unroll
+            for (int i = 3 * g; i < 3 * g + 3; ++i) ld2(s + 1, i);
+          }
+#pragma unroll
+          for (int rb = 0; rb < 2; ++rb)
+#pragma unroll
+            for (int j = 0; j < 4; ++j)
+              acc2[rb][j] = __builtin_amdgcn_mfma_f32_32x32x16_bf16(a2[s & 1][rb][qa[g]], b2[s & 1][j][qb[g]],
+                                                                    acc2[rb][j], 0, 0, 0);
+        }
+      }
+    }
+    barrier_lds();
+
+    {
+      const int wl = lane + launder(), r32 = wl & 31, hh = wl >> 5;
+      int dpb[4], dvm[4];
+    #pragma unroll
+      for (int cb = 0; cb < 4; ++cb) {
+        const int n = 32 * cb + r32, a = n / Wa, b = n - a * Wa;
+        dpb[cb] = a * p.w + b;
+        dvm[cb] = 0;
+    #pragma unroll
+        for (int t = 0; t < 4; ++t)
+          if (n < NA && a + (t >> 1) < p.h && b + (t & 1) < p.w) dvm[cb] |= 1 << t;
+      }
+      auto dpix = [&](int cb, int t) { return (dvm[cb] >> t) & 1 ? dpb[cb] + (t >> 1) * p.w + (t & 1) : kVbDN - 1; };
+      f32x16 acc[4];
+#pragma unroll
+      for (int cb = 0; cb < 4; ++cb)
+#pragma unroll
+        for (int e = 0; e < 16; ++e) acc[cb][e] = 0.f;
+      bf16x8 a[3][3], b[2][4][3];
+      const bf16x8* Ws = p.Ws + (size_t)wave * 16 * 3 * 64 + wl;
+      auto lda = [&](int s) {
+#pragma unroll
+        for (int q = 0; q < 3; ++q) a[s % 3][q] = Ws[(s * 3 + q) * 64];
+      };
+      auto ldb = [&](int s, int i) {
+        const int t = s >> 2, ch = 16 * (s & 3) + 8 * hh, cb = i / 3, q = i % 3;
+        b[s & 1][cb][q] = *reinterpret_cast<const bf16x8*>(dpl + q * kVbDB + vb_dofs(dpix(cb, t), ch));
+      };
+      lda(0);
+      lda(1);
+#pragma unroll
+      for (int i = 0; i < 12; ++i) ldb(0, i);
+      for (int i = tid; i < (16 * KS1 - P1) * 12; i += 256) {
+        const int q = i % 3, r = i / 3;
+        *reinterpret_cast<u32x4*>(tpl + q * kVbTB + (P1 + (r >> 2)) * 64 + (r & 3) * 16) = u32x4{0u, 0u, 0u, 0u};
+      }
+#pragma unroll
+      for (int s = 0; s < 16; ++s) {
+        if (s + 2 < 16) lda(s + 2);
+        __builtin_amdgcn_sched_barrier(0);
+        constexpr int qa[6] = {2, 0, 1, 1, 0, 0}, qb[6] = {0, 2, 1, 0, 1, 0};
+#pragma unroll
+        for (int g = 0; g < 6; ++g) {
+          if (s + 1 < 16) {
+            ldb(s + 1, 2 * g);
+            ldb(s + 1, 2 * g + 1);
+          }
+#pragma unroll
+          for (int cb = 0; cb < 4; ++cb)
+            acc[cb] = __builtin_amdgcn_mfma_f32_32x32x16_bf16(a[s % 3][qa[g]], b[s & 1][cb][qb[g]], acc[cb], 0, 0, 0);
+        }
+        __builtin_amdgcn_sched_barrier(0);
+      }
+#pragma unroll
+      for (int cb = 0; cb < 4; ++cb) {
+        const int n = 32 * cb + r32, a0 = n / Wa, b0 = n - a0 * Wa, y1 = 2 * a0 + py, x1 = 2 * b0 + px;
+        if (n < NA && y1 < p.H1 && x1 < p.W1) {
+          const int p1 = y1 * p.W1 + x1;
+#pragma unroll
+          for (int g = 0; g < 4; ++g) {
+            const f32x4 v = {acc[cb][4 * g], acc[cb][4 * g + 1], acc[cb][4 * g + 2], acc[cb][4 * g + 3]};
+#pragma unroll
+            for (int e = 0; e < 4; ++e) bsum[4 * g + e] += v[e];
+            vq_commit4(tpl + p1 * 64 + (8 * g + 4 * hh) * 2, kVbTB, v);
+            if constexpr (DY1) *reinterpret_cast<f32x4*>(p.dy1 + ((size_t)f * P1 + p1) * 32 + 8 * g + 4 * hh) = v;
+          }
+        }
+      }
+    }
+    barrier_lds();
+
+    const int tl = tid + launder();
+    build(tl);
+    const int fn = f + (int)gridDim.x;
+    if (fn < p.F) fetch(fn, tl);
+    barrier_lds();
+
+    {
+      const int wl = lane + launder(), r32 = wl & 31, hh = wl >> 5, tq = (wl & 15) >> 2, tp = wl & 3;
+      int oy[2], ox[2];
+#pragma unroll
+      for (int u = 0; u < 2; ++u) {
+        const int pix = 8 * hh + tq + 4 * u;
+        oy[u] = pix / p.W1;
+        ox[u] = pix - oy[u] * p.W1;
+      }
+      const int ao = 8 * hh * 64 + tq * 64 + ((r32 & 16) + 4 * tp) * 2;
+      const int kxo = (((r32 & 16) >> 2) + tp) * 8;
+      auto frags = [&](int s, bf16x8 (&a1)[3], bf16x8 (&b1)[2]) {
+#pragma unroll
+        for (int q = 0; q < 3; ++q) a1[q] = vb_tr(tpl + q * kVbTB, ao + 16 * s * 64, ao + 16 * s * 64 + 4 * 64);
+        int xo[2];
+#pragma unroll
+        for (int u = 0; u < 2; ++u) {
+          const bool ok = 16 * s + 8 * hh + tq + 4 * u < P1;
+          xo[u] = ok ? (4 * oy[u] * Wp + 4 * ox[u]) * 8 + kxo : kxo;
+        }
+#pragma unroll
+        for (int j = 0; j < 2; ++j) b1[j] = vb_tr(xim, xo[0] + (2 * wave + j) * Wp * 8, xo[1] + (2 * wave + j) * Wp * 8);
+#pragma unroll
+        for (int u = 0; u < 2; ++u) {
+          ox[u] += 16;
+          if (ox[u] >= p.W1) { ox[u] -= p.W1; ++oy[u]; }
+          if (ox[u] >= p.W1) { ox[u] -= p.W1; ++oy[u]; }
+        }
+      };
+      bf16x8 ac[3], bc[2];
+      frags(0, ac, bc);
+      for (int s = 0; s < KS1; ++s) {
+        bf16x8 an[3], bn[2];
+        if (s + 1 < KS1) frags(s + 1, an, bn);
+#pragma unroll
+        for (int q = 2; q >= 0; --q)
+#pragma unroll
+          for (int j = 0; j < 2; ++j) acc1[j] = __builtin_amdgcn_mfma_f32_32x32x16_bf16(ac[q], bc[j], acc1[j], 0, 0, 0);
+#pragma unroll
+        for (int q = 0; q < 3; ++q) ac[q] = an[q];
+        bc[0] = bn[0];
+        bc[1] = bn[1];
+      }
+    }
+    barrier_lds();
+  }
+
+  float* pt = p.part + (size_t)blockIdx.x * kVbPart;
+#pragma unroll
+  for (int rb = 0; rb < 2; ++rb)
+#pragma unroll
+    for (int j = 0; j < 4; ++j)
+#pragma unroll
+      for (int g = 0; g < 4; ++g)
+#pragma unroll
+        for (int e = 0; e < 4; ++e)
+          pt[(32 * rb + 8 * g + 4 * hh + e) * 512 + 32 * (4 * wave + j) + r32] = acc2[rb][j][4 * g + e];
+#pragma unroll
+  for (int j = 0; j < 2; ++j)
+#pragma unroll
+    for (int g = 0; g < 4; ++g)
+#pragma unroll
+      for (int e = 0; e < 4; ++e)
+        pt[32768 + (8 * g + 4 * hh + e) * 256 + 32 * (2 * wave + j) + r32] = acc1[j][4 * g + e];
+  float* red = reinterpret_cast<float*>(lds);
+#pragma unroll
+  for (int i = 0; i < 16; ++i) red[(wave * 64 + lane) * 16 + i] = bsum[i];
+  __syncthreads();
+  if (tid < 32) {
+    const int g = tid >> 3, h2 = (tid >> 2) & 1, e = tid & 3;
+    float t = 0.f;
+    for (int w = 0; w < 4; ++w)
+      for (int l = 0; l < 32; ++l) t += red[(w * 64 + 32 * h2 + l) * 16 + 4 * g + e];
+    pt[40960 + tid] = t;
+  }
+}
+
+inline int vbwd_f32_groups(int F, int cus, size_t part_bytes, int max_groups = 0) {
+  const int rounds = (F + cus - 1) / cus;
+  int g = (F + rounds - 1) / rounds;
+  g = (int)std::min<size_t>((size_t)g, part_bytes / ((size_t)kVbPart * 4));
+  if (max_groups > 0) g = std::min(g, max_groups);
+  return g;
+}
+
+inline hipError_t vision_bwd_frames_f32(const VisBwdF32Params& p, int nwg, float* gW2, float* gW1, float* gb1,
+                                        hipStream_t st) {
+  if (!vbwd_f32_fits(p.H, p.W, p.H1, p.W1, p.h, p.w) || p.F < 1 || nwg < 1) return hipErrorInvalidValue;
+  if (p.dy1) hipLaunchKernelGGL((k_vision_bwd_f32<true>), dim3(nwg), dim3(256), 0, st, p);
+  else hipLaunchKernelGGL((k_vision_bwd_f32<false>), dim3(nwg), dim3(256), 0, st, p);
+  hipLaunchKernelGGL(k_vbwd_reduce, dim3((kVbPart + 63) / 64), dim3(256), 0, st, p.part, nwg, gW2, gW1, gb1);
+  return hipGetLastError();
+}
+
+}
diff --git a/towards-interpretable-reinforcement-learning-using-attention-augmented-agents-replication_amd/runtime.py b/towards-interpretable-reinforcement-learning-using-attention-augmented-agents-replication_amd/runtime.py
--- a/towards-interpretable-reinforcement-learning-using-attention-augmented-agents-replication_amd/runtime.py
+++ b/towards-interpretable-reinforcement-learning-using-attention-augmented-agents-replication_amd/runtime.py
@@ -379,6 +379,26 @@
                                                 N.ptr(frames), N.ptr(xp), N.ptr(y1), N.ptr(out), N.stream_ptr(dev)),
                 "vision_enc_f32_fwd")
         return xp, y1, out
+
+    def backward(self, packed, frames, dy2, y1, xp, max_groups: int = 0):
+        dev = self.device
+        want = torch.uint8 if self.u8 else torch.float32
+        if frames.dtype != want or tuple(frames.shape) != (self.N, self.H, self.W, 3):
+            raise ValueError(f"frames must be {want} of shape {(self.N, self.H, self.W, 3)}")
+        if dy2.dtype != torch.float32 or tuple(dy2.shape) != (self.N, self.h * self.w, 64):
+            raise ValueError("dy2 must be float32 (N, h*w, 64)")
+        frames, dy2 = frames.to(dev).contiguous(), dy2.to(dev).contiguous()
+        ws_bytes = self.lib.aaa_vision_enc_f32_workspace_bytes(ctypes.byref(self.desc))
+        if not ws_bytes:
+            N.check(-1, "vision_enc_f32 workspace")
+        grads = torch.empty(32 * 3 * 64 + 32 + 64 * 32 * 16 + 64, device=dev)
+        dy1 = torch.full((self.N, self.H1, self.W1, 32), float("nan"), device=dev)
+        ws = torch.empty(ws_bytes, dtype=torch.uint8, device=dev)
+        fused = ctypes.c_int(-1)
+        N.check(self.lib.aaa_vision_enc_f32_bwd(ctypes.byref(self.desc), N.ptr(packed), N.ptr(frames), N.ptr(dy2),
+                                                N.ptr(y1), N.ptr(xp), N.ptr(dy1), N.ptr(grads), ctypes.byref(fused),
+                                                int(max_groups), N.ptr(ws), N.stream_ptr(dev)), "vision_enc_f32_bwd")
+        return grads, dy1, bool(fused.value)
 
 
 class ActorRunner:
```

After: 243,200 frames/s (median of 6 runs). 1.02x the previous value.
